# skhu101/SHERF

Hardware: NVIDIA B200
Metric: ray_samples_per_sec (higher is better)
Workload: dtype bf16x3 (bf16 hi/lo split products on tcgen05 kind::f16, 16 significand bits per operand, fp32 accumulate) in every linear layer

## Files before the change

### include/sherf_b200.h

```cpp
#ifndef SHERF_B200_H
#define SHERF_B200_H

#include <stddef.h>
#include <stdint.h>

#ifdef __cplusplus
extern "C" {
#endif

#define SHERF_ABI_VERSION 5
#if defined(__GNUC__)
#define SHERF_API __attribute__((visibility("default")))
#else
#define SHERF_API
#endif
#define SHERF_NUM_JOINTS 24
#define SHERF_NUM_LEVELS 3

enum {
  SHERF_OK = 0,
  SHERF_E_INVALID = -1,
  SHERF_E_SCRATCH = -2,
  SHERF_E_CUDA = -3,
  SHERF_E_UNSUPPORTED = -4
// ... 168 lines not shown
                                                  const SherfInputGrads* grad_inputs, void* scratch, size_t scratch_bytes, void* stream,
                                                  int64_t n_points);

SHERF_API int sherf_depth_range(const SherfRays* rays, float* min_out , float* max_out ,
                      void* scratch, size_t scratch_bytes, void* stream);

SHERF_API int sherf_generate_rays(const double* K, const double* R, const double* T, int32_t H, int32_t W, const double* bounds,
                                  float* origins, float* dirs, float* near_out, float* far_out, uint8_t* mask_at_box ,
                                  void* stream);

#define SHERF_SPARSE_CONVS 13
typedef struct SherfSparseConv {
  const float* weight;
  const float *bn_weight, *bn_bias, *bn_mean, *bn_var;
  int32_t c_in, c_out;
  int32_t kind;
  int32_t reserved;
} SherfSparseConv;
typedef struct SherfSparseEncoder { SherfSparseConv conv[SHERF_SPARSE_CONVS]; } SherfSparseEncoder;

SHERF_API size_t sherf_sparse_encoder_scratch_bytes(int32_t n_voxels, const int32_t* out_sh );
SHERF_API int sherf_sparse_encode(const SherfSparseEncoder* enc, const int32_t* coord, const float* feat, int32_t n,
                                  const int32_t* out_sh , float* vol1, float* vol2, float* vol3, void* scratch,
                                  size_t scratch_bytes, void* stream);

typedef struct SherfSparseEncoderGrads {
  float* weight[SHERF_SPARSE_CONVS];
  float* bn_weight[SHERF_SPARSE_CONVS];
  float* bn_bias[SHERF_SPARSE_CONVS];
} SherfSparseEncoderGrads;
SHERF_API size_t sherf_sparse_encoder_train_scratch_bytes(int32_t n_voxels, const int32_t* out_sh );
SHERF_API int sherf_sparse_encode_train(const SherfSparseEncoder* enc, const int32_t* coord, const float* feat, int32_t n,
                                        const int32_t* out_sh , float* vol1, float* vol2, float* vol3, float* batch_stats,
                                        int32_t* row_counts, int32_t use_running_stats, void* scratch, size_t scratch_bytes, void* stream);
SHERF_API int sherf_sparse_encode_backward(const SherfSparseEncoder* enc, const int32_t* coord, int32_t n, const int32_t* out_sh ,
                                           const float* g_vol1, const float* g_vol2, const float* g_vol3, const SherfSparseEncoderGrads* grads,
                                           float* g_feat, int32_t use_running_stats , void* scratch, size_t scratch_bytes,
                                           void* stream);

typedef struct SherfObservation {
  SherfPose obs;
  SherfPose canonical;
  const float* obs_vertices;
  const float* t_vertices;
  const float* obs_K;
  const float* obs_R;
  const float* obs_T;
  const int32_t* faces;
  const int32_t* last_face;
  int32_t n_faces;
  int32_t reserved;
  const float* obs_img;
  int32_t img_h, img_w;
  const float* obs_feat;
  int32_t feat_ch, feat_h, feat_w;
  int32_t reserved2;
  const float *proj_w, *proj_b;
} SherfObservation;

SHERF_API size_t sherf_observation_scratch_bytes(int32_t n_verts);
SHERF_API int sherf_prepare_observation(const SherfSmplModel* smpl, const SherfObservation* obs, float* vert_feat, int32_t* coord,
                                        uint8_t* vertex_mask, float* bounds, int32_t* out_sh_host, float* canonical_out, void* scratch,
                                        size_t scratch_bytes, void* stream);

SHERF_API int sherf_prepare_observation_backward(const SherfSmplModel* smpl, const SherfObservation* obs, const float* g_vert_feat,
                                                 float* g_proj_w, float* g_proj_b, float* g_obs_feat, void* scratch, size_t scratch_bytes,
                                                 void* stream);

SHERF_API int sherf_debug_sample_importance(const SherfRays* rays, const float* weights, const float* u, float* t_fine_out,
                                            int32_t* bins_out , void* stream);

SHERF_API int sherf_debug_linear(int precision, const float* A, int lda, const float* W, const float* bias, float* Y, int ldy,
                                 int M, int N, int K, int act, void* scratch, size_t scratch_bytes, void* stream);

SHERF_API void sherf_debug_set_trace(long long* device_buf);

SHERF_API const char* sherf_last_error(void);
SHERF_API int sherf_abi_version(void);
SHERF_API int64_t sherf_last_launch_count(void);
SHERF_API int64_t sherf_last_importance_point_count(void);
SHERF_API void sherf_set_profiling(int enabled);
SHERF_API float sherf_last_stage_ms(int stage);
SHERF_API float sherf_last_host_us(int part);

#ifdef __cplusplus
}
#endif
#endif
```

### sherf_b200/_lib.py

```python
from __future__ import annotations

import ctypes as C
import os

from . import build as _build

c_float_p = C.c_void_p
c_int_p = C.c_void_p

MLP_FP32, MLP_TF32, MLP_TF32X3, MLP_BF16X3 = 0, 1, 2, 3
ABI_VERSION = 5


class SherfSmplModel(C.Structure):
    _fields_ = [('v_template', c_float_p), ('shapedirs', c_float_p), ('posedirs', c_float_p), ('j_regressor', c_float_p),
                ('weights', c_float_p), ('parents', C.c_int32 * 24), ('n_verts', C.c_int32)]


class SherfPose(C.Structure):
    _fields_ = [('poses', c_float_p), ('shapes', c_float_p), ('R', c_float_p), ('Th', c_float_p)]


class SherfFrame(C.Structure):
    _fields_ = [('target', SherfPose), ('canonical', SherfPose), ('obs', SherfPose), ('vertices', c_float_p),
                ('t_vertices', c_float_p), ('t_world_bounds', c_float_p), ('obs_K', c_float_p), ('obs_R', c_float_p),
                ('obs_T', c_float_p), ('sp_bounds', c_float_p), ('out_sh', C.c_int32 * 3)]


class SherfScene(C.Structure):
    _fields_ = [('planes', c_float_p), ('plane_ch', C.c_int32), ('plane_h', C.c_int32), ('plane_w', C.c_int32),
                ('obs_img', c_float_p), ('img_h', C.c_int32), ('img_w', C.c_int32),
                ('obs_feat', c_float_p), ('feat_ch', C.c_int32), ('feat_h', C.c_int32), ('feat_w', C.c_int32),
                ('vol', c_float_p * 3), ('vol_ch', C.c_int32 * 3), ('vol_dim', (C.c_int32 * 3) * 3)]


class SherfWeights(C.Structure):
    _fields_ = [('proj_w', c_float_p), ('proj_b', c_float_p), ('reproj_w', c_float_p), ('reproj_b', c_float_p),
                ('ln1_w', c_float_p), ('ln1_b', c_float_p), ('qkv_w', c_float_p), ('attn_out_w', c_float_p),
                ('attn_out_b', c_float_p), ('ln2_w', c_float_p), ('ln2_b', c_float_p), ('ff1_w', c_float_p),
                ('ff1_b', c_float_p), ('ff2_w', c_float_p), ('ff2_b', c_float_p), ('pts_w', c_float_p * 8),
                ('pts_b', c_float_p * 8), ('alpha_w', c_float_p), ('alpha_b', c_float_p), ('feature_w', c_float_p),
                ('feature_b', c_float_p), ('views_w', c_float_p), ('views_b', c_float_p), ('rgb_w', c_float_p),
                ('rgb_b', c_float_p)]


class SherfWeightGrads(C.Structure):
    _fields_ = list(SherfWeights._fields_)


class SherfOutGrads(C.Structure):
    _fields_ = [('rgb', c_float_p), ('depth', c_float_p), ('acc', c_float_p)]


class SherfInputGrads(C.Structure):
    _fields_ = [('planes', c_float_p), ('obs_feat', c_float_p), ('vol', c_float_p * 3)]


class SherfRays(C.Structure):
    _fields_ = [('origins', c_float_p), ('dirs', c_float_p), ('near_', c_float_p), ('far_', c_float_p),
                ('n_rays', C.c_int32), ('n_samples', C.c_int32), ('n_importance', C.c_int32), ('reserved', C.c_int32)]


class SherfOptions(C.Structure):
    _fields_ = [('white_back', C.c_int32), ('mlp_precision', C.c_int32), ('depth_clamp_min', C.c_float),
                ('depth_clamp_max', C.c_float), ('use_external_clamp', C.c_int32), ('density_noise', c_float_p),
                ('importance_u', c_float_p), ('density_noise_importance', c_float_p), ('weights_version', C.c_uint64), ('scene_version', C.c_uint64)]


class SherfOut(C.Structure):
    _fields_ = [('rgb', c_float_p), ('depth', c_float_p), ('acc', c_float_p)]


class SherfDebug(C.Structure):
    _fields_ = [('sample_vid', c_int_p), ('point_sample', c_int_p), ('point_vid3', c_int_p), ('point_can', c_float_p),
                ('point_cdir', c_float_p), ('point_uv', c_float_p), ('point_feat', c_float_p), ('point_tok', c_float_p),
                ('point_sigma', c_float_p), ('point_rgb', c_float_p), ('max_points', C.c_int64), ('max_feat_points', C.c_int64),
                ('coarse_weights', c_float_p), ('fine_depths', c_float_p), ('fine_bins', c_int_p), ('fine_sample_vid', c_int_p),
                ('fine_sigma', c_float_p), ('fine_rgb', c_float_p)]


class SherfSparseConv(C.Structure):
    _fields_ = [('weight', c_float_p), ('bn_weight', c_float_p), ('bn_bias', c_float_p), ('bn_mean', c_float_p), ('bn_var', c_float_p),
                ('c_in', C.c_int32), ('c_out', C.c_int32), ('kind', C.c_int32), ('reserved', C.c_int32)]


class SherfSparseEncoder(C.Structure):
    _fields_ = [('conv', SherfSparseConv * 13)]


class SherfSparseEncoderGrads(C.Structure):
    _fields_ = [('weight', c_float_p * 13), ('bn_weight', c_float_p * 13), ('bn_bias', c_float_p * 13)]


class SherfObservation(C.Structure):
    _fields_ = [('obs', SherfPose), ('canonical', SherfPose), ('obs_vertices', c_float_p), ('t_vertices', c_float_p), ('obs_K', c_float_p),
                ('obs_R', c_float_p), ('obs_T', c_float_p), ('faces', c_int_p), ('last_face', c_int_p), ('n_faces', C.c_int32),
                ('reserved', C.c_int32), ('obs_img', c_float_p), ('img_h', C.c_int32), ('img_w', C.c_int32), ('obs_feat', c_float_p),
                ('feat_ch', C.c_int32), ('feat_h', C.c_int32), ('feat_w', C.c_int32), ('reserved2', C.c_int32), ('proj_w', c_float_p),
                ('proj_b', c_float_p)]


EXPORTS = ['sherf_render_backward_after_forward', 'sherf_sparse_encoder_train_scratch_bytes', 'sherf_sparse_encode_train', 'sherf_sparse_encode_backward', 'sherf_prepare_observation_backward', 'sherf_backward_scratch_bytes', 'sherf_render_backward', 'sherf_smpl_vertices', 'sherf_count_survivors', 'sherf_observation_scratch_bytes', 'sherf_prepare_observation', 'sherf_debug_set_trace', 'sherf_sparse_encoder_scratch_bytes', 'sherf_sparse_encode', 'sherf_generate_rays', 'sherf_debug_sample_importance', 'sherf_debug_linear', 'sherf_scratch_bytes', 'sherf_render_forward', 'sherf_lbs_transforms', 'sherf_depth_range', 'sherf_last_error',
           'sherf_abi_version', 'sherf_last_launch_count', 'sherf_last_importance_point_count', 'sherf_set_profiling', 'sherf_last_stage_ms', 'sherf_last_host_us']

_lib = None


def lib_path() -> str:
    return _build.LIB_PATH


def load():
    global _lib
    if _lib is not None:
        return _lib
    path = lib_path()
    if not os.path.exists(path):
        raise RuntimeError(f'{path} not found: build it with `python -m sherf_b200.build` (or __graft_entry__.build()); '
                           'sherf_b200 has no CPU or PyTorch fallback')
    lib = C.CDLL(path)
    lib.sherf_scratch_bytes.restype = C.c_size_t
    lib.sherf_scratch_bytes.argtypes = [C.POINTER(SherfScene), C.c_int32, C.c_int32, C.c_int32, C.c_int32]
    lib.sherf_render_forward.restype = C.c_int
    lib.sherf_render_forward.argtypes = [C.POINTER(SherfSmplModel), C.POINTER(SherfFrame), C.POINTER(SherfScene),
                                         C.POINTER(SherfWeights), C.POINTER(SherfRays), C.POINTER(SherfOptions),
                                         C.POINTER(SherfOut), C.POINTER(SherfDebug), C.c_void_p, C.c_size_t, C.c_void_p,
                                         C.POINTER(C.c_int64)]
    lib.sherf_backward_scratch_bytes.restype = C.c_size_t
    lib.sherf_backward_scratch_bytes.argtypes = [C.POINTER(SherfScene), C.c_int32, C.c_int32, C.c_int32]
    lib.sherf_render_backward.restype = C.c_int
    lib.sherf_render_backward.argtypes = [C.POINTER(SherfSmplModel), C.POINTER(SherfFrame), C.POINTER(SherfScene),
                                          C.POINTER(SherfWeights), C.POINTER(SherfRays), C.POINTER(SherfOptions),
                                          C.POINTER(SherfOutGrads), C.POINTER(SherfWeightGrads), C.POINTER(SherfInputGrads),
                                          C.c_void_p, C.c_size_t, C.c_void_p, C.POINTER(C.c_int64)]
    lib.sherf_render_backward_after_forward.restype = C.c_int
    lib.sherf_render_backward_after_forward.argtypes = lib.sherf_render_backward.argtypes[:-1] + [C.c_int64]
    lib.sherf_count_survivors.restype = C.c_int
    lib.sherf_count_survivors.argtypes = [C.POINTER(SherfSmplModel), C.POINTER(SherfFrame), C.POINTER(SherfScene), C.POINTER(SherfRays),
                                          C.POINTER(SherfOptions), C.c_void_p, C.c_size_t, C.c_void_p, C.POINTER(C.c_int64)]
    lib.sherf_smpl_vertices.restype = C.c_int
    lib.sherf_smpl_vertices.argtypes = [C.POINTER(SherfSmplModel), C.POINTER(SherfPose), C.c_void_p, C.c_void_p, C.c_void_p, C.c_size_t, C.c_void_p]
    lib.sherf_lbs_transforms.restype = C.c_int
    lib.sherf_lbs_transforms.argtypes = [C.POINTER(SherfSmplModel), C.POINTER(SherfPose), C.c_void_p, C.c_void_p, C.c_size_t,
                                         C.c_void_p]
    lib.sherf_depth_range.restype = C.c_int
    lib.sherf_depth_range.argtypes = [C.POINTER(SherfRays), C.POINTER(C.c_float), C.POINTER(C.c_float), C.c_void_p, C.c_size_t,
                                      C.c_void_p]
    lib.sherf_debug_linear.restype = C.c_int
    lib.sherf_debug_linear.argtypes = [C.c_int, C.c_void_p, C.c_int, C.c_void_p, C.c_void_p, C.c_void_p, C.c_int, C.c_int, C.c_int, C.c_int,
                                       C.c_int, C.c_void_p, C.c_size_t, C.c_void_p]
    lib.sherf_debug_sample_importance.restype = C.c_int
    lib.sherf_debug_sample_importance.argtypes = [C.POINTER(SherfRays), C.c_void_p, C.c_void_p, C.c_void_p, C.c_void_p, C.c_void_p]
    lib.sherf_generate_rays.restype = C.c_int
    lib.sherf_generate_rays.argtypes = [C.POINTER(C.c_double), C.POINTER(C.c_double), C.POINTER(C.c_double), C.c_int32, C.c_int32,
                                        C.POINTER(C.c_double), C.c_void_p, C.c_void_p, C.c_void_p, C.c_void_p, C.c_void_p, C.c_void_p]
    lib.sherf_sparse_encoder_scratch_bytes.restype = C.c_size_t
    lib.sherf_sparse_encoder_scratch_bytes.argtypes = [C.c_int32, C.POINTER(C.c_int32)]
    lib.sherf_sparse_encode.restype = C.c_int
    lib.sherf_sparse_encode.argtypes = [C.POINTER(SherfSparseEncoder), C.c_void_p, C.c_void_p, C.c_int32, C.POINTER(C.c_int32), C.c_void_p, C.c_void_p,
                                        C.c_void_p, C.c_void_p, C.c_size_t, C.c_void_p]
    lib.sherf_sparse_encoder_train_scratch_bytes.restype = C.c_size_t
    lib.sherf_sparse_encoder_train_scratch_bytes.argtypes = [C.c_int32, C.POINTER(C.c_int32)]
    lib.sherf_sparse_encode_train.restype = C.c_int
    lib.sherf_sparse_encode_train.argtypes = [C.POINTER(SherfSparseEncoder), C.c_void_p, C.c_void_p, C.c_int32, C.POINTER(C.c_int32), C.c_void_p,
                                              C.c_void_p, C.c_void_p, C.c_void_p, C.c_void_p, C.c_int32, C.c_void_p, C.c_size_t, C.c_void_p]
    lib.sherf_sparse_encode_backward.restype = C.c_int
    lib.sherf_sparse_encode_backward.argtypes = [C.POINTER(SherfSparseEncoder), C.c_void_p, C.c_int32, C.POINTER(C.c_int32), C.c_void_p, C.c_void_p,
                                                 C.c_void_p, C.POINTER(SherfSparseEncoderGrads), C.c_void_p, C.c_int32, C.c_void_p, C.c_size_t, C.c_void_p]
    lib.sherf_prepare_observation_backward.restype = C.c_int
    lib.sherf_prepare_observation_backward.argtypes = [C.POINTER(SherfSmplModel), C.POINTER(SherfObservation), C.c_void_p, C.c_void_p, C.c_void_p,
                                                       C.c_void_p, C.c_void_p, C.c_size_t, C.c_void_p]
    lib.sherf_observation_scratch_bytes.restype = C.c_size_t
    lib.sherf_observation_scratch_bytes.argtypes = [C.c_int32]
    lib.sherf_prepare_observation.restype = C.c_int
    lib.sherf_prepare_observation.argtypes = [C.POINTER(SherfSmplModel), C.POINTER(SherfObservation), C.c_void_p, C.c_void_p, C.c_void_p,
                                              C.c_void_p, C.POINTER(C.c_int32), C.c_void_p, C.c_void_p, C.c_size_t, C.c_void_p]
    lib.sherf_debug_set_trace.argtypes = [C.c_void_p]
    lib.sherf_last_error.restype = C.c_char_p
    lib.sherf_abi_version.restype = C.c_int
    lib.sherf_last_launch_count.restype = C.c_int64
    lib.sherf_last_importance_point_count.restype = C.c_int64
    lib.sherf_set_profiling.argtypes = [C.c_int]
    lib.sherf_last_stage_ms.restype = C.c_float
    lib.sherf_last_stage_ms.argtypes = [C.c_int]
    lib.sherf_last_host_us.restype = C.c_float
    lib.sherf_last_host_us.argtypes = [C.c_int]
    if lib.sherf_abi_version() != ABI_VERSION:
        raise RuntimeError('libsherf_b200.so ABI version mismatch')
    _lib = lib
    return lib


def check(rc: int):
    if rc != 0:
        raise RuntimeError(f'sherf_b200 error {rc}: {load().sherf_last_error().decode()}')
```

### sherf_b200/csrc/api.cu

```cuda
#include "common.cuh"
#include "stages.cuh"
#include <cstdarg>
#include <cstdio>
#include <cstring>
#include <cstdlib>
#include <vector>
#include <chrono>

namespace sherf {

thread_local LaunchCounter g_launches;
thread_local bool g_pack_plan_only = false;
static thread_local char g_err[512] = "";
static thread_local int64_t g_last_launches = 0;
static thread_local int64_t g_last_fine_points = 0;
static thread_local int g_profiling = 0;
static thread_local float g_stage_ms[8] = {0, 0, 0, 0, 0, 0, 0, 0};
static thread_local float g_host_us[4] = {0, 0, 0, 0};
static inline double now_us() { return std::chrono::duration<double, std::micro>(std::chrono::steady_clock::now().time_since_epoch()).count(); }

void set_error(const char* fmt, ...) {
  va_list ap;
  va_start(ap, fmt);
  vsnprintf(g_err, sizeof(g_err), fmt, ap);
  va_end(ap);
}

constexpr int kMaxCell = 1 << 18;
static size_t chunk_cap_limit() {
  static size_t cap = 0;
  if (!cap) {
    const char* e = getenv("SHERF_CHUNK_CAP");
    const long v = e ? atol(e) : 0;
    cap = v >= 128 ? (size_t)(v / 128 * 128) : (size_t)(1 << 19);
  }
  return cap;
}

struct Arena {
  char* base; size_t size; size_t off; bool dry;
  template <typename T> T* take(size_t n) {
    off = (off + 255) & ~(size_t)255;
    T* p = dry ? nullptr : reinterpret_cast<T*>(base + off);
    off += n * sizeof(T);
    return p;
  }
};

struct Layout {
  FrameTables ft;
  float* planes_cl; float* feat_cl; float* vol_cl[3];
  int* sample_vid; int* ray_count; int* block_sums; int* ray_start; int64_t* total;
  int* point_sample; int* point_vid;
  float* sigma; float* rgb;
  float* fine_depths; int* sample_vid_f; int* ray_count_f; int* ray_start_f; int64_t* total_f; int* point_sample_f; int* point_vid_f;
  float* sigma_f; float* rgb_f;
  float* packed_w;
  float* canon_w;
  unsigned char* fused_blob; float* fused_bias; float* xf_blob; float* ff_blob;
  unsigned char* pp_blob; float* pp_bias; unsigned char* pp_xv;
  unsigned char* xb_blob; unsigned char* fr_blob;
  float* chunk;
  float* gather2;
  float* lbs_joints; float* lbs_pf;
};

static int chunk_cap(int N, int S, int SF) {
  const size_t NS = (size_t)N * (S > SF ? S : SF);
  return (int)((NS < chunk_cap_limit()) ? ((NS + 127) / 128 * 128) : chunk_cap_limit());
}

static size_t carve(Arena& a, const SherfScene& sc, int N, int S, int SF, int V, Layout& L) {
  const size_t NS = (size_t)N * S, NF = (size_t)N * SF;
  FrameTables& ft = L.ft;
  ft.fc = a.take<FrameConst>(1);
  ft.A = a.take<float>(3 * kJoints * 16);
  ft.joints = a.take<float>(3 * kJoints * 3);
  ft.posefeat = a.take<float>(3 * kPoseFeat);
  ft.poff = a.take<float>((size_t)3 * V * 3);
  ft.soff = a.take<float>((size_t)2 * V * 3);
  ft.verts_smpl = a.take<float>((size_t)V * 3);
  ft.T1 = a.take<VertexWarp>(V);
  ft.T3 = a.take<VertexWarp>(V);
  ft.g1_cell_start = a.take<int>(kMaxCell + 1);
  ft.g3_cell_start = a.take<int>(kMaxCell + 1);
  ft.g_cursor = a.take<int>((size_t)2 * kMaxCell);
  ft.g_block_sums = a.take<int>((size_t)2 * (kMaxCell / 1024 + 2));
  ft.g_total = a.take<int64_t>(2);
  ft.g1_verts = a.take<float4>(V);
  ft.g3_verts = a.take<float4>(V);
  ft.g1_occ = a.take<unsigned char>(kMaxCell);
  ft.maxcell = kMaxCell;
  L.lbs_joints = a.take<float>(kJoints * 3);
  L.lbs_pf = a.take<float>(kPoseFeat);
  L.planes_cl = a.take<float>((size_t)3 * sc.plane_ch * sc.plane_h * sc.plane_w);
  L.feat_cl = a.take<float>((size_t)sc.feat_ch * sc.feat_h * sc.feat_w);
  for (int l = 0; l < 3; ++l)
    L.vol_cl[l] = a.take<float>((size_t)sc.vol_ch[l] * sc.vol_dim[l][0] * sc.vol_dim[l][1] * sc.vol_dim[l][2]);
  L.sample_vid = a.take<int>(NS);
  L.ray_count = a.take<int>(N);
  L.block_sums = a.take<int>((size_t)N / 1024 + 2);
  L.ray_start = a.take<int>((size_t)N + 1);
  L.total = a.take<int64_t>(1);
  L.point_sample = a.take<int>(NS);
  L.point_vid = a.take<int>(NS);
  L.sigma = a.take<float>(NS);
  L.rgb = a.take<float>(NS * 3);
  L.fine_depths = nullptr; L.sample_vid_f = nullptr; L.ray_count_f = nullptr; L.ray_start_f = nullptr; L.total_f = nullptr;
  L.point_sample_f = nullptr; L.point_vid_f = nullptr; L.sigma_f = nullptr; L.rgb_f = nullptr;
  if (SF > 0) {
    L.fine_depths = a.take<float>(NF);
    L.sample_vid_f = a.take<int>(NF);
    L.ray_count_f = a.take<int>(N);
    L.ray_start_f = a.take<int>((size_t)N + 1);
    L.total_f = a.take<int64_t>(1);
    L.point_sample_f = a.take<int>(NF);
    L.point_vid_f = a.take<int>(NF);
    L.sigma_f = a.take<float>(NF);
    L.rgb_f = a.take<float>(NF * 3);
  }
  L.packed_w = a.take<float>(packed_weight_floats());
  L.canon_w = a.take<float>(canonical_weight_floats());
  L.fused_blob = a.take<unsigned char>(fused_blob_bytes());
  L.fused_bias = a.take<float>(10 * 144);
  L.xf_blob = a.take<float>(xformer_blob_floats());
  L.ff_blob = a.take<float>(fusion_blob_floats());
  const int cap = chunk_cap(N, S, SF);
  L.chunk = a.take<float>(chunk_buffer_floats(cap));
  L.pp_blob = a.take<unsigned char>(pp_blob_bytes());
  L.pp_bias = a.take<float>(10 * 128);
  L.pp_xv = a.take<unsigned char>(pp_xv_bytes(cap));
  L.gather2 = a.take<float>((size_t)cap * (288 + 192 + 8));
  L.xb_blob = a.take<unsigned char>(xformer_bf16_blob_bytes());
  L.fr_blob = a.take<unsigned char>(front_blob_bytes());
  return a.off;
}

struct StageTimer {
  struct Span { int stage; cudaEvent_t a, b; cudaStream_t s; };
  std::vector<Span> spans; bool on = false; cudaStream_t st = nullptr;
  std::vector<int> open_stack;
  static std::vector<cudaEvent_t>& pool() { static thread_local std::vector<cudaEvent_t> p; return p; }
  size_t used = 0;
  cudaEvent_t get_event() {
    auto& p = pool();
    if (used == p.size()) { cudaEvent_t e; cudaEventCreate(&e); p.push_back(e); }
    return p[used++];
  }
  void init(bool enable, cudaStream_t s) { on = enable; st = s; used = 0; }
  void begin(int stage, cudaStream_t on_stream = nullptr) {
    if (!on) return;
    Span sp; sp.stage = stage; sp.s = on_stream ? on_stream : st;
    sp.a = get_event(); sp.b = get_event();
    cudaEventRecord(sp.a, sp.s);
    spans.push_back(sp);
    open_stack.push_back((int)spans.size() - 1);
  }
  void end() {
    if (!on || open_stack.empty()) return;
    cudaEventRecord(spans[open_stack.back()].b, spans[open_stack.back()].s);
    open_stack.pop_back();
  }
  void finish() {
    if (!on) return;
    for (int i = 0; i < 8; ++i) g_stage_ms[i] = 0.f;
    cudaStreamSynchronize(st);
    for (auto& sp : spans) {
      float ms = 0.f;
      cudaEventElapsedTime(&ms, sp.a, sp.b);
      g_stage_ms[sp.stage] += ms;
    }
    spans.clear();
  }
};

static thread_local StageTimer* g_tm = nullptr;

struct PackTag { const void* base = nullptr; size_t need = 0; uint64_t version = 0; int precision = -1; int dev = -1; uint64_t scene = 0; };
static thread_local PackTag g_pack_tag;

static int64_t* pinned_counts() {
  static thread_local int64_t* p = nullptr;
  if (!p && cudaHostAlloc((void**)&p, 4 * sizeof(int64_t), cudaHostAllocDefault) != cudaSuccess) p = nullptr;
  return p;
}

static cudaEvent_t count_event(int which) {
  static thread_local cudaEvent_t ev[2] = {nullptr, nullptr};
  static thread_local int dev = -1;
  int d = 0;
  if (cudaGetDevice(&d) != cudaSuccess) return nullptr;
  if (d != dev) { ev[0] = ev[1] = nullptr; dev = d; }
  if (!ev[which] && cudaEventCreateWithFlags(&ev[which], cudaEventDisableTiming) != cudaSuccess) ev[which] = nullptr;
  return ev[which];
}

struct SideStream {
  cudaStream_t s = nullptr; cudaEvent_t fork = nullptr, ldone = nullptr, gdone[2] = {nullptr, nullptr}, mdone[2] = {nullptr, nullptr}; int dev = -1;
  int ensure() {
    int d = 0;
    if (cudaGetDevice(&d) != cudaSuccess) return -1;
    if (s && d == dev) return 0;
    dev = d;
    int lo = 0, hi = 0;
    cudaDeviceGetStreamPriorityRange(&lo, &hi);
    if (cudaStreamCreateWithPriority(&s, cudaStreamNonBlocking, hi) != cudaSuccess) return -1;
    cudaEventCreateWithFlags(&fork, cudaEventDisableTiming);
    cudaEventCreateWithFlags(&ldone, cudaEventDisableTiming);
    for (int i = 0; i < 2; ++i) { cudaEventCreateWithFlags(&gdone[i], cudaEventDisableTiming); cudaEventCreateWithFlags(&mdone[i], cudaEventDisableTiming); }
    return 0;
  }
};
static thread_local SideStream g_side;
static void fill_gather_params(GatherParams& G, const SherfRays& rays, const SherfFrame& frame, const SherfScene& scene, const Layout& L) {
  G.origins = rays.origins; G.dirs = rays.dirs; G.nearv = rays.near_; G.farv = rays.far_; G.S = rays.n_samples; G.depths = nullptr;
  G.point_sample = L.point_sample; G.point_vid = L.point_vid; G.p0 = 0; G.np = 0; G.dc = DevCount{nullptr, 0, 0};
  G.fc = L.ft.fc; G.T1 = L.ft.T1; G.T3 = L.ft.T3; G.g3_start = L.ft.g3_cell_start; G.g3_verts = L.ft.g3_verts;
  G.t_vertices = getenv("SHERF_KNN3_UNSEEDED") ? nullptr : frame.t_vertices;
  G.planes_cl = L.planes_cl; G.plane_h = scene.plane_h; G.plane_w = scene.plane_w;
  G.feat_cl = L.feat_cl; G.feat_h = scene.feat_h; G.feat_w = scene.feat_w; G.feat_ch = scene.feat_ch;
  G.img = scene.obs_img; G.img_h = scene.img_h; G.img_w = scene.img_w;
  for (int l = 0; l < 3; ++l) {
    G.vol_cl[l] = L.vol_cl[l]; G.vol_ch[l] = scene.vol_ch[l];
    G.vol_d[l] = scene.vol_dim[l][0]; G.vol_h[l] = scene.vol_dim[l][1]; G.vol_w[l] = scene.vol_dim[l][2];
  }
  G.comb = nullptr; G.f3raw = nullptr; G.geo = nullptr;
  G.g_planes_cl = nullptr; G.g_feat_cl = nullptr; G.g_vol_cl[0] = G.g_vol_cl[1] = G.g_vol_cl[2] = nullptr;
  G.dbg_vid3 = nullptr; G.dbg_can = nullptr; G.dbg_cdir = nullptr; G.dbg_uv = nullptr; G.dbg_feat = nullptr; G.dbg_max = 0; G.dbg_feat_max = 0;
}

struct BwdLayout {
  float* out;
  float* dsig; float* drgb;
  float* g_planes_cl; float* g_feat_cl; float* g_vol_cl[3];
  float* canon_w; float* canon_bwd;
  float* chunk; int bcap;
};
static int bwd_chunk_cap(int N, int S) {
  const char* e = getenv("SHERF_BWD_CHUNK_CAP");
  const long v = e ? atol(e) : 0;
  const int cap = v >= 128 ? (int)(v / 128 * 128) : (1 << 20);
  const size_t NS = (size_t)N * S;
  return (int)(NS < (size_t)cap ? (NS + 127) / 128 * 128 : (size_t)cap);
}
static size_t carve_backward(Arena& a, const SherfScene& sc, int N, int S, int V, Layout& L, BwdLayout& B, size_t* fwd_need) {
  const size_t f = carve(a, sc, N, S, 0, V, L);
  if (fwd_need) *fwd_need = f;
  const size_t NS = (size_t)N * S;
  B.out = a.take<float>((size_t)5 * N);
  B.dsig = a.take<float>(NS);
  B.drgb = a.take<float>(NS * 3);
  B.g_planes_cl = a.take<float>((size_t)3 * sc.plane_ch * sc.plane_h * sc.plane_w);
  B.g_feat_cl = a.take<float>((size_t)sc.feat_ch * sc.feat_h * sc.feat_w);
  for (int l = 0; l < 3; ++l) B.g_vol_cl[l] = a.take<float>((size_t)sc.vol_ch[l] * sc.vol_dim[l][0] * sc.vol_dim[l][1] * sc.vol_dim[l][2]);
  B.canon_w = a.take<float>(canonical_weight_floats());
  B.canon_bwd = a.take<float>(canonical_bwd_weight_floats());
  B.bcap = bwd_chunk_cap(N, S);
  B.chunk = a.take<float>(bwd_chunk_floats(B.bcap));
  return a.off;
}

static void nested_begin(int stage) { if (g_tm) g_tm->begin(stage); }
static void nested_end() { if (g_tm) g_tm->end(); }

}

using namespace sherf;

extern "C" {

int sherf_abi_version(void) { return SHERF_ABI_VERSION; }
const char* sherf_last_error(void) { return g_err; }
int64_t sherf_last_launch_count(void) { return g_last_launches; }
int64_t sherf_last_importance_point_count(void) { return g_last_fine_points; }
void sherf_set_profiling(int enabled) { g_profiling = enabled; }
float sherf_last_stage_ms(int stage) { return (stage >= 0 && stage < 8) ? g_stage_ms[stage] : 0.f; }
float sherf_last_host_us(int part) { return (part >= 0 && part < 4) ? g_host_us[part] : 0.f; }

size_t sherf_scratch_bytes(const SherfScene* scene, int32_t n_rays, int32_t n_samples, int32_t n_importance, int32_t n_verts) {
  if (!scene || n_rays <= 0 || n_samples < 2 || n_importance < 0 || n_verts <= 0) return 0;
  Arena a{nullptr, 0, 0, true};
  Layout L;
  return carve(a, *scene, n_rays, n_samples, n_importance, n_verts, L) + 512;
}

static int validate(const SherfSmplModel* smpl, const SherfFrame* fr, const SherfScene* sc, const SherfWeights* w,
                    const SherfRays* rays, const SherfOptions* opts, const SherfOut* out) {
  if (!smpl || !fr || !sc || !w || !rays || !opts || !out) { set_error("null argument struct"); return SHERF_E_INVALID; }
  if (rays->n_rays <= 0 || rays->n_samples < 2 || rays->n_samples > 256) {
    set_error("n_rays must be > 0 and 2 <= n_samples <= 256 (got %d, %d)", rays->n_rays, rays->n_samples);
    return SHERF_E_INVALID;
  }
  if ((int64_t)rays->n_rays * rays->n_samples >= (1LL << 31)) { set_error("n_rays * n_samples must be < 2^31"); return SHERF_E_INVALID; }
  if (rays->n_importance < 0 || rays->n_importance > 256) { set_error("n_importance must be in 0..256 (got %d)", rays->n_importance); return SHERF_E_INVALID; }
  if (rays->n_importance > 0) {
    if (rays->n_samples < 3) { set_error("the importance pass needs n_samples >= 3 (sample_pdf bins, renderer.py:498-499)"); return SHERF_E_INVALID; }
    if (!opts->importance_u) { set_error("n_importance > 0 needs SherfOptions.importance_u (the torch.rand draws of renderer.py:526)"); return SHERF_E_INVALID; }
    const int64_t smax = rays->n_samples > rays->n_importance ? rays->n_samples : rays->n_importance;
    if ((int64_t)rays->n_rays * smax >= (1LL << 30)) { set_error("n_rays * max(n_samples, n_importance) must be < 2^30 with the importance pass"); return SHERF_E_INVALID; }
  }
  if (sc->plane_ch != 32 || sc->feat_ch != 64 || sc->vol_ch[0] != 32 || sc->vol_ch[1] != 64 || sc->vol_ch[2] != 96) {
    set_error("unsupported channel counts (planes %d, feat %d, volumes %d/%d/%d; expected 32, 64, 32/64/96)", sc->plane_ch,
              sc->feat_ch, sc->vol_ch[0], sc->vol_ch[1], sc->vol_ch[2]);
    return SHERF_E_UNSUPPORTED;
  }
  if (opts->mlp_precision < SHERF_MLP_FP32 || opts->mlp_precision > SHERF_MLP_BF16X3) { set_error("unknown mlp_precision %d", opts->mlp_precision); return SHERF_E_UNSUPPORTED; }
  if (!rays->origins || !rays->dirs || !rays->near_ || !rays->far_ || !out->rgb || !out->depth || !out->acc || !sc->planes ||
      !sc->obs_img || !sc->obs_feat || !sc->vol[0] || !sc->vol[1] || !sc->vol[2] || !smpl->weights || !smpl->posedirs) {
    set_error("null device pointer in arguments");
    return SHERF_E_INVALID;
  }
  {
    const SherfPose* poses[3] = {&fr->target, &fr->canonical, &fr->obs};
    bool ok = fr->vertices && fr->t_vertices && fr->t_world_bounds && fr->obs_K && fr->obs_R && fr->obs_T && fr->sp_bounds && smpl->v_template &&
              smpl->shapedirs && smpl->j_regressor;
    for (int i = 0; i < 3; ++i) ok = ok && poses[i]->poses && poses[i]->shapes;
    ok = ok && fr->target.R && fr->target.Th && fr->obs.R && fr->obs.Th;
    const float* const* wp = reinterpret_cast<const float* const*>(w);
    for (size_t i = 0; i < sizeof(SherfWeights) / sizeof(const float*); ++i) ok = ok && wp[i] != nullptr;
    if (!ok) { set_error("null device pointer in SherfFrame / SherfSmplModel / SherfWeights"); return SHERF_E_INVALID; }
  }
  return SHERF_OK;
}

#define RC(x) do { int _rc = (x); if (_rc) return _rc; } while (0)

int sherf_render_forward(const SherfSmplModel* smpl, const SherfFrame* frame, const SherfScene* scene,
                         const SherfWeights* weights, const SherfRays* rays, const SherfOptions* opts, const SherfOut* out,
                         const SherfDebug* dbg, void* scratch, size_t scratch_bytes, void* stream, int64_t* n_points_out) {
  g_err[0] = 0;
  const double t_enter = now_us();
  RC(validate(smpl, frame, scene, weights, rays, opts, out));
  const int N = rays->n_rays, S = rays->n_samples, SF = rays->n_importance, V = smpl->n_verts;
  cudaStream_t st = (cudaStream_t)stream;
  Arena a{(char*)scratch, scratch_bytes, 0, false};
  const size_t mis = ((size_t)a.base) & 255;
  if (mis) { a.base += 256 - mis; a.size -= 256 - mis; }
  Layout L;
  const size_t need = carve(a, *scene, N, S, SF, V, L);
  if (!scratch || need > a.size) { set_error("scratch arena too small: need %zu bytes, have %zu", need, scratch_bytes); return SHERF_E_SCRATCH; }
  g_launches.n = 0;
  g_last_fine_points = 0;
  StageTimer tm;
  tm.init(g_profiling != 0, st);
  g_tm = &tm;
  struct Guard {
    cudaStream_t st; bool forked = false, joined = false;
    ~Guard() {
      g_tm = nullptr;
      if (forked && !joined && g_side.s) { cudaEventRecord(g_side.ldone, g_side.s); cudaStreamWaitEvent(st, g_side.ldone, 0); }
    }
  } guard;
  guard.st = st;

  const bool side = !getenv("SHERF_NO_PROLOGUE_OVERLAP") && g_side.ensure() == 0;
  cudaStream_t ls = side ? g_side.s : st;
  tm.begin(0);
  RC(run_prologue_frame(*frame, L.ft, st));
  if (side) { SHERF_CUDA_OK(cudaEventRecord(g_side.fork, st)); SHERF_CUDA_OK(cudaStreamWaitEvent(ls, g_side.fork, 0)); guard.forked = true; }
  RC(run_prologue_cull(*smpl, *frame, *rays, *opts, L.ft, st));
// ... 82 lines not shown
    G.S = Sn; G.depths = depths; G.point_sample = point_sample; G.point_vid = point_vid; G.p0 = p0; G.np = np; G.dc = dc;
    G.comb = cbi.comb; G.f3raw = cbi.f3raw; G.geo = cbi.geo;
    G.dbg_vid3 = d ? d->point_vid3 : nullptr; G.dbg_can = d ? d->point_can : nullptr;
    G.dbg_cdir = d ? d->point_cdir : nullptr; G.dbg_uv = d ? d->point_uv : nullptr;
    G.dbg_feat = d ? d->point_feat : nullptr; G.dbg_max = d ? d->max_points : 0;
    G.dbg_feat_max = d ? d->max_feat_points : 0;
    if (overlap && ci >= 2) SHERF_CUDA_OK(cudaStreamWaitEvent(gs, g_side.mdone[bsel], 0));
    tm.begin(2, gs);
    if (fplan.fr_blob) RC(run_front_fused(G, *weights, fplan.fr_blob, cbi.tok, gs));
    else RC(run_point_gather(G, gs));
    tm.end();
    if (overlap) { SHERF_CUDA_OK(cudaEventRecord(g_side.gdone[bsel], gs)); SHERF_CUDA_OK(cudaStreamWaitEvent(st, g_side.gdone[bsel], 0)); }
    tm.begin(3);
    RC(run_mlp(opts->mlp_precision, *weights, pw, cw, use_fused ? &fplan : nullptr, cbi, np, p0, sigma_out, rgb_out, d ? d->point_tok : nullptr,
               d ? d->max_points : 0, st, nested_begin, nested_end, dc));
    tm.end();
    if (overlap) SHERF_CUDA_OK(cudaEventRecord(g_side.mdone[bsel], st));
    return SHERF_OK;
  };
  auto run_points = [&](const int* point_sample, const int* point_vid, int64_t Pn, int64_t first_p0, int Sn, const float* depths, float* sigma_out,
                        float* rgb_out, const SherfDebug* d) -> int {
    const bool overlap = first_p0 == 0 && Pn > cb.cap && getenv("SHERF_OVERLAP") && g_side.ensure() == 0;
    cudaStream_t gs = overlap ? g_side.s : st;
    if (overlap) { SHERF_CUDA_OK(cudaEventRecord(g_side.fork, st)); SHERF_CUDA_OK(cudaStreamWaitEvent(gs, g_side.fork, 0)); }
    int ci = (int)(first_p0 / cb.cap);
    for (int64_t p0 = first_p0; p0 < Pn; p0 += cb.cap, ++ci) {
      const int np = (int)((Pn - p0 < cb.cap) ? (Pn - p0) : cb.cap);
      RC(issue_chunk(point_sample, point_vid, p0, np, Sn, depths, sigma_out, rgb_out, d, DevCount{nullptr, 0, 0}, ci, overlap, gs));
    }
    return SHERF_OK;
  };
  const bool async_first = fplan.fr_blob && fplan.xb_blob && use_pp && !dbg && !getenv("SHERF_SYNC_FIRST_CHUNK");
  if (side) { SHERF_CUDA_OK(cudaStreamWaitEvent(st, g_side.ldone, 0)); guard.joined = true; }
  if (async_first)
    RC(issue_chunk(L.point_sample, L.point_vid, 0, cb.cap, S, nullptr, L.sigma, L.rgb, nullptr, DevCount{L.total, 0, cb.cap}, 0, false, st));
  const double t_sync0 = now_us();
  SHERF_CUDA_OK(cudaEventSynchronize(ev_cnt0));
  const int64_t P = hcount[0];
  const double t_sync1 = now_us();
  if (n_points_out) *n_points_out = P;
  if (dbg && dbg->point_sample && P > 0)
    SHERF_CUDA_OK(cudaMemcpyAsync(dbg->point_sample, L.point_sample, sizeof(int) * (size_t)(P < dbg->max_points ? P : dbg->max_points),
                                  cudaMemcpyDeviceToDevice, st));
  RC(run_points(L.point_sample, L.point_vid, P, async_first ? cb.cap : 0, S, nullptr, L.sigma, L.rgb, dbg));
  if (dbg && P > 0) {
    const size_t cnt = (size_t)(P < dbg->max_points ? P : dbg->max_points);
    if (dbg->point_sigma) SHERF_CUDA_OK(cudaMemcpyAsync(dbg->point_sigma, L.sigma, sizeof(float) * cnt, cudaMemcpyDeviceToDevice, st));
    if (dbg->point_rgb) SHERF_CUDA_OK(cudaMemcpyAsync(dbg->point_rgb, L.rgb, sizeof(float) * 3 * cnt, cudaMemcpyDeviceToDevice, st));
  }

  if (SF == 0) {
    tm.begin(4);
    RC(run_composite(*rays, L.ft.fc, L.ray_start, L.point_sample, L.sigma, L.rgb, opts->density_noise, opts->white_back, *out, st));
    tm.end();
  } else {
    tm.begin(4);
    RC(run_importance_sample(*rays, L.ray_start, L.point_sample, L.sigma, opts->density_noise, nullptr, opts->importance_u, L.fine_depths,
                             dbg ? dbg->fine_bins : nullptr, dbg ? dbg->coarse_weights : nullptr, st));
    tm.end();
    tm.begin(1);
    int* vid_f = (dbg && dbg->fine_sample_vid) ? dbg->fine_sample_vid : L.sample_vid_f;
    RC(run_cull(*rays, SF, L.fine_depths, L.ft, vid_f, L.ray_count_f, L.block_sums, L.ray_start_f, L.total_f, L.point_sample_f, L.point_vid_f, st));
    tm.end();
    SHERF_CUDA_OK(cudaMemcpyAsync(&hcount[1], L.total_f, sizeof(int64_t), cudaMemcpyDeviceToHost, st));
    SHERF_CUDA_OK(cudaEventRecord(ev_cnt1, st));
    if (async_first)
      RC(issue_chunk(L.point_sample_f, L.point_vid_f, 0, cb.cap, SF, L.fine_depths, L.sigma_f, L.rgb_f, nullptr, DevCount{L.total_f, 0, cb.cap}, 0, false, st));
    SHERF_CUDA_OK(cudaEventSynchronize(ev_cnt1));
    const int64_t PF = hcount[1];
    if (n_points_out) *n_points_out = P + PF;
    g_last_fine_points = PF;
    RC(run_points(L.point_sample_f, L.point_vid_f, PF, async_first ? cb.cap : 0, SF, L.fine_depths, L.sigma_f, L.rgb_f, nullptr));
    if (dbg) {
      if (dbg->fine_depths) SHERF_CUDA_OK(cudaMemcpyAsync(dbg->fine_depths, L.fine_depths, sizeof(float) * (size_t)N * SF, cudaMemcpyDeviceToDevice, st));
      RC(run_dense_taps(L.point_sample_f, L.sigma_f, L.rgb_f, PF, (int64_t)N * SF, dbg->fine_sigma, dbg->fine_rgb, st));
    }
    tm.begin(4);
    RC(run_composite_merged(*rays, L.ft.fc, sample_vid, L.ray_start, L.sigma, L.rgb, opts->density_noise, L.fine_depths, vid_f, L.ray_start_f,
                            L.sigma_f, L.rgb_f, opts->density_noise_importance, opts->white_back, *out, st));
    tm.end();
  }
  tm.finish();
  g_last_launches = g_launches.n;
  { const double t_exit = now_us(); g_host_us[0] = (float)(t_sync0 - t_enter); g_host_us[1] = (float)(t_sync1 - t_sync0); g_host_us[2] = (float)(t_exit - t_sync1); g_host_us[3] = (float)(t_exit - t_enter); }
  return SHERF_OK;
}

size_t sherf_backward_scratch_bytes(const SherfScene* scene, int32_t n_rays, int32_t n_samples, int32_t n_verts) {
  if (!scene || n_rays <= 0 || n_samples < 2 || n_verts <= 0) return 0;
  Arena a{nullptr, 0, 0, true};
  Layout L;
  BwdLayout B;
  return carve_backward(a, *scene, n_rays, n_samples, n_verts, L, B, nullptr) + 512;
}

static int render_backward_impl(const SherfSmplModel* smpl, const SherfFrame* frame, const SherfScene* scene, const SherfWeights* weights,
                                const SherfRays* rays, const SherfOptions* opts, const SherfOutGrads* grad_out, const SherfWeightGrads* grad_weights,
                                const SherfInputGrads* grad_inputs, void* scratch, size_t scratch_bytes, void* stream, int64_t* n_points_out,
                                int64_t forward_points );

int sherf_render_backward(const SherfSmplModel* smpl, const SherfFrame* frame, const SherfScene* scene, const SherfWeights* weights,
                          const SherfRays* rays, const SherfOptions* opts, const SherfOutGrads* grad_out, const SherfWeightGrads* grad_weights,
                          const SherfInputGrads* grad_inputs, void* scratch, size_t scratch_bytes, void* stream, int64_t* n_points_out) {
  return render_backward_impl(smpl, frame, scene, weights, rays, opts, grad_out, grad_weights, grad_inputs, scratch, scratch_bytes, stream, n_points_out, -1);
}

int sherf_render_backward_after_forward(const SherfSmplModel* smpl, const SherfFrame* frame, const SherfScene* scene, const SherfWeights* weights,
                                        const SherfRays* rays, const SherfOptions* opts, const SherfOutGrads* grad_out,
                                        const SherfWeightGrads* grad_weights, const SherfInputGrads* grad_inputs, void* scratch, size_t scratch_bytes,
                                        void* stream, int64_t n_points) {
  if (n_points < 0) { g_err[0] = 0; set_error("n_points must be the survivor count the forward reported"); return SHERF_E_INVALID; }
  return render_backward_impl(smpl, frame, scene, weights, rays, opts, grad_out, grad_weights, grad_inputs, scratch, scratch_bytes, stream, nullptr, n_points);
}

}

static int render_backward_impl(const SherfSmplModel* smpl, const SherfFrame* frame, const SherfScene* scene, const SherfWeights* weights,
                                const SherfRays* rays, const SherfOptions* opts, const SherfOutGrads* grad_out, const SherfWeightGrads* grad_weights,
                                const SherfInputGrads* grad_inputs, void* scratch, size_t scratch_bytes, void* stream, int64_t* n_points_out,
                                int64_t forward_points) {
  g_err[0] = 0;
  if (!smpl || !frame || !scene || !weights || !rays || !opts || !grad_out || !scratch) { set_error("null argument"); return SHERF_E_INVALID; }
  if (rays->n_importance != 0) {
    set_error("sherf_render_backward covers the coarse pass only (n_importance must be 0; the reference's fine pass cannot execute, SURVEY a13)");
    return SHERF_E_UNSUPPORTED;
  }
  const int N = rays->n_rays, S = rays->n_samples, V = smpl->n_verts;
  if (N <= 0 || S < 2 || V <= 0) { set_error("bad sizes"); return SHERF_E_INVALID; }
  cudaStream_t st = (cudaStream_t)stream;
  Arena a{(char*)scratch, scratch_bytes, 0, false};
  const size_t mis = ((size_t)a.base) & 255;
  if (mis) { a.base += 256 - mis; a.size -= 256 - mis; }
  Layout L;
  BwdLayout B;
  size_t fwd_need = 0;
  const size_t need = carve_backward(a, *scene, N, S, V, L, B, &fwd_need);
  if (need > a.size) { set_error("backward scratch arena too small: need %zu bytes, have %zu", need, scratch_bytes); return SHERF_E_SCRATCH; }

  SherfOut fout; fout.rgb = B.out; fout.depth = B.out + (size_t)3 * N; fout.acc = B.out + (size_t)4 * N;
  int64_t P = forward_points;
  int64_t launches = 0;
  if (forward_points < 0) {
    RC(sherf_render_forward(smpl, frame, scene, weights, rays, opts, &fout, nullptr, a.base, fwd_need + 256, stream, &P));
    launches = g_launches.n;
  } else if (forward_points > (int64_t)N * S) { set_error("n_points exceeds n_rays * n_samples"); return SHERF_E_INVALID; }
  if (n_points_out) *n_points_out = P;
  g_launches.n = 0;

  SherfWeightGrads gw;
  if (grad_weights) gw = *grad_weights; else memset(&gw, 0, sizeof(gw));
  {
    float* const* gp = reinterpret_cast<float* const*>(&gw);
    const int n_out[20] = {96, 32, 32, 144, 32, 32, 32, 32, 128, 128, 128, 128, 128, 128, 128, 128, 1, 128, 64, 3};
    const int n_in[20] = {192, 96, 0, 32, 48, 0, 32, 32, 71, 128, 128, 128, 128, 199, 128, 128, 128, 128, 187, 64};
    size_t sizes[39]; int k = 0;
    auto wb = [&](int layer, bool bias) { sizes[k++] = (size_t)n_out[layer] * (n_in[layer] ? n_in[layer] : 1); if (bias) sizes[k++] = n_out[layer]; };
    wb(0, true); wb(1, true);
    sizes[k++] = 32; sizes[k++] = 32;
    wb(3, false); wb(4, true);
    sizes[k++] = 32; sizes[k++] = 32;
    wb(6, true); wb(7, true);
    for (int i = 0; i < 8; ++i) sizes[k++] = (size_t)128 * n_in[8 + i];
    for (int i = 0; i < 8; ++i) sizes[k++] = 128;
    wb(16, true); wb(17, true); wb(18, true); wb(19, true);
    if (k != 39 || sizeof(SherfWeightGrads) != 39 * sizeof(float*)) { set_error("internal: weight table mismatch"); return SHERF_E_INVALID; }
    for (int i = 0; i < 39; ++i)
      if (gp[i]) SHERF_CUDA_OK(cudaMemsetAsync(gp[i], 0, sizes[i] * sizeof(float), st));
  }
  const bool want_planes = grad_inputs && grad_inputs->planes, want_feat = grad_inputs && grad_inputs->obs_feat;
  bool want_vol[3];
  for (int l = 0; l < 3; ++l) want_vol[l] = grad_inputs && grad_inputs->vol[l];
  const size_t plane = (size_t)scene->plane_ch * scene->plane_h * scene->plane_w;
  if (want_planes) SHERF_CUDA_OK(cudaMemsetAsync(B.g_planes_cl, 0, 3 * plane * sizeof(float), st));
  if (want_feat) SHERF_CUDA_OK(cudaMemsetAsync(B.g_feat_cl, 0, (size_t)scene->feat_ch * scene->feat_h * scene->feat_w * sizeof(float), st));
  size_t vol_n[3];
  for (int l = 0; l < 3; ++l) {
    vol_n[l] = (size_t)scene->vol_ch[l] * scene->vol_dim[l][0] * scene->vol_dim[l][1] * scene->vol_dim[l][2];
    if (want_vol[l]) SHERF_CUDA_OK(cudaMemsetAsync(B.g_vol_cl[l], 0, vol_n[l] * sizeof(float), st));
  }

  if (P > 0) {
    PackedWeights pw;
    g_pack_plan_only = false;
    RC(run_pack_weights(*weights, L.packed_w, pw, st));
    CanonWeights cw;
    CanonBwdWeights cbw;
    RC(run_pack_canonical(*weights, B.canon_w, cw, st));
    RC(run_pack_canonical_bwd(*weights, B.canon_bwd, cbw, st));
    RC(run_composite_backward(*rays, L.ft.fc, L.ray_start, L.point_sample, L.sigma, L.rgb, opts->density_noise, opts->white_back, grad_out->rgb,
                              grad_out->depth, grad_out->acc, B.dsig, B.drgb, st));
    BwdChunk bc;
    carve_bwd_chunk(B.chunk, B.bcap, bc);
    GatherParams G;
    fill_gather_params(G, *rays, *frame, *scene, L);
    for (int64_t p0 = 0; p0 < P; p0 += B.bcap) {
      const int np = (int)((P - p0 < B.bcap) ? (P - p0) : B.bcap);
      RC(run_backward_chunk(*weights, pw, cw, cbw, gw, G, bc, np, p0, L.rgb, B.dsig, B.drgb, st));
      GatherParams Gs = G;
      Gs.g_planes_cl = want_planes ? B.g_planes_cl : nullptr;
      Gs.g_feat_cl = want_feat ? B.g_feat_cl : nullptr;
      for (int l = 0; l < 3; ++l) Gs.g_vol_cl[l] = want_vol[l] ? B.g_vol_cl[l] : nullptr;
      RC(run_backward_chunk_inputs(*weights, cbw, Gs, bc, np, p0, st));
    }
  }
  if (want_planes)
    for (int k = 0; k < 3; ++k)
      RC(run_from_channels_last(B.g_planes_cl + k * plane, grad_inputs->planes + k * plane, scene->plane_ch, (int64_t)scene->plane_h * scene->plane_w, st));
  if (want_feat) RC(run_from_channels_last(B.g_feat_cl, grad_inputs->obs_feat, scene->feat_ch, (int64_t)scene->feat_h * scene->feat_w, st));
  for (int l = 0; l < 3; ++l)
    if (want_vol[l])
      RC(run_from_channels_last(B.g_vol_cl[l], grad_inputs->vol[l], scene->vol_ch[l], (int64_t)(vol_n[l] / scene->vol_ch[l]), st));
  g_last_launches = launches + g_launches.n;
  return SHERF_OK;
}

extern "C" {

int sherf_count_survivors(const SherfSmplModel* smpl, const SherfFrame* frame, const SherfScene* scene, const SherfRays* rays, const SherfOptions* opts,
                          void* scratch, size_t scratch_bytes, void* stream, int64_t* n_points_out) {
  g_err[0] = 0;
  if (!smpl || !frame || !scene || !rays || !opts || !scratch || !n_points_out) { set_error("null argument"); return SHERF_E_INVALID; }
  if (rays->n_rays <= 0 || rays->n_samples < 2 || rays->n_samples > 256 || !rays->origins || !rays->dirs || !rays->near_ || !rays->far_) {
    set_error("bad rays"); return SHERF_E_INVALID;
  }
  const int N = rays->n_rays, S = rays->n_samples, SF = rays->n_importance, V = smpl->n_verts;
  cudaStream_t st = (cudaStream_t)stream;
  Arena a{(char*)scratch, scratch_bytes, 0, false};
  const size_t mis = ((size_t)a.base) & 255;
  if (mis) { a.base += 256 - mis; a.size -= 256 - mis; }
  Layout L;
  const size_t need = carve(a, *scene, N, S, SF, V, L);
  if (need > a.size) { set_error("scratch arena too small: need %zu bytes, have %zu", need, scratch_bytes); return SHERF_E_SCRATCH; }
  g_launches.n = 0;
  RC(run_prologue_frame(*frame, L.ft, st));
  RC(run_prologue_cull(*smpl, *frame, *rays, *opts, L.ft, st));
  RC(run_cull(*rays, S, nullptr, L.ft, L.sample_vid, L.ray_count, L.block_sums, L.ray_start, L.total, L.point_sample, L.point_vid, st));
  int64_t* hcount = pinned_counts();
  if (!hcount) { set_error("cudaHostAlloc failed for the survivor-count words"); return SHERF_E_CUDA; }
  SHERF_CUDA_OK(cudaMemcpyAsync(&hcount[2], L.total, sizeof(int64_t), cudaMemcpyDeviceToHost, st));
  SHERF_CUDA_OK(cudaStreamSynchronize(st));
  *n_points_out = hcount[2];
  g_last_launches = g_launches.n;
  return SHERF_OK;
}

int sherf_debug_sample_importance(const SherfRays* rays, const float* weights, const float* u, float* t_fine_out, int32_t* bins_out,
                                  void* stream) {
  g_err[0] = 0;
  if (!rays || !weights || !u || !t_fine_out || !rays->near_ || !rays->far_) { set_error("null argument"); return SHERF_E_INVALID; }
  if (rays->n_rays <= 0 || rays->n_samples < 3 || rays->n_samples > 256 || rays->n_importance < 1 || rays->n_importance > 256) {
    set_error("need n_rays > 0, 3 <= n_samples <= 256, 1 <= n_importance <= 256");
    return SHERF_E_INVALID;
  }
  g_launches.n = 0;
  RC(run_importance_sample(*rays, nullptr, nullptr, nullptr, nullptr, weights, u, t_fine_out, bins_out, nullptr, (cudaStream_t)stream));
  g_last_launches = g_launches.n;
  return SHERF_OK;
}

int sherf_generate_rays(const double* K, const double* R, const double* T, int32_t H, int32_t W, const double* bounds, float* origins,
                        float* dirs, float* near_out, float* far_out, uint8_t* mask_at_box, void* stream) {
  g_err[0] = 0;
  if (!K || !R || !T || !bounds || !origins || !dirs || !near_out || !far_out) { set_error("null argument"); return SHERF_E_INVALID; }
  if (H <= 0 || W <= 0 || (int64_t)H * W >= (1LL << 31)) { set_error("bad image size %d x %d", H, W); return SHERF_E_INVALID; }
  g_launches.n = 0;
  RC(run_generate_rays(K, R, T, H, W, bounds, origins, dirs, near_out, far_out, mask_at_box, (cudaStream_t)stream));
  g_last_launches = g_launches.n;
  return SHERF_OK;
}

size_t sherf_sparse_encoder_scratch_bytes(int32_t n_voxels, const int32_t* out_sh) {
  if (n_voxels <= 0 || !out_sh || out_sh[0] <= 0 || out_sh[1] <= 0 || out_sh[2] <= 0) return 0;
  return sparse_encoder_scratch_bytes(n_voxels, out_sh);
}

int sherf_sparse_encode(const SherfSparseEncoder* enc, const int32_t* coord, const float* feat, int32_t n, const int32_t* out_sh, float* vol1,
                        float* vol2, float* vol3, void* scratch, size_t scratch_bytes, void* stream) {
// ... 182 lines not shown
```

### sherf_b200/csrc/common.cuh

```cuda
#pragma once
#include <cuda_runtime.h>
#include <stdint.h>
#include <stddef.h>
#include <string.h>
#include "../../include/sherf_b200.h"

namespace sherf {

constexpr int kJoints = 24;
constexpr int kPoseFeat = 207;
constexpr float kPi2 = 1.57079632679489661923f;

struct GridDesc {
  float origin[3];
  float inv_cell;
  float cell;
  int dim[3];
  int ncell;
};

struct __align__(16) VertexWarp {
  float Rinv[9];
  float t[3];
  float off0[3];
  float off1[3];
  float off2[3];
  float Af[12];
  float pad[3];
};
static_assert(sizeof(VertexWarp) == 36 * 4, "VertexWarp must be 144 B");

struct FrameConst {
  float R_tgt[9], Th_tgt[3];
  float Rinv_obs[9], Th_obs[3];
  float camR[9], camT[3], camK[9];
  float twb_min[3], twb_max[3];
  float spb_min[3];
  float out_sh[3];
  GridDesc g1, g3;
  int dmin_bits, dmax_bits;
  float dmin, dmax;
};

__host__ __device__ inline int float_to_ordered(float f) {
#ifdef __CUDA_ARCH__
  int i = __float_as_int(f);
#else
  int i; memcpy(&i, &f, 4);
#endif
  return i >= 0 ? i : i ^ 0x7fffffff;
}
__device__ inline float ordered_to_float(int i) { return __int_as_float(i >= 0 ? i : i ^ 0x7fffffff); }

__device__ __forceinline__ float sample_depth(float nearv, float farv, int i, int S) {
  float step = __fdiv_rn((float)i, (float)(S - 1));
  return __fadd_rn(nearv, __fmul_rn(step, __fsub_rn(farv, nearv)));
}
__device__ __forceinline__ float mul_add_sep(float a, float b, float c) {
  return __fadd_rn(c, __fmul_rn(a, b));
}
__device__ __forceinline__ void rowvec_mat3(const float p[3], const float* __restrict__ M, float out[3]) {
#pragma unroll
  for (int j = 0; j < 3; ++j)
    out[j] = __fmaf_rn(p[2], M[6 + j], __fmaf_rn(p[1], M[3 + j], __fmul_rn(p[0], M[j])));
}
__device__ __forceinline__ float dist2_xyz(float qx, float qy, float qz, float vx, float vy, float vz) {
  float dx = __fsub_rn(qx, vx), dy = __fsub_rn(qy, vy), dz = __fsub_rn(qz, vz);
  return __fadd_rn(__fadd_rn(__fmul_rn(dx, dx), __fmul_rn(dy, dy)), __fmul_rn(dz, dz));
}
__device__ __forceinline__ int grid_coord(float x, float origin, float inv_cell, int dim) {
  int c = (int)floorf((x - origin) * inv_cell);
  return c;
}

__device__ __forceinline__ void mat3_vec(const float* __restrict__ M, const float v[3], float out[3]) {
#pragma unroll
  for (int i = 0; i < 3; ++i) out[i] = M[3 * i] * v[0] + M[3 * i + 1] * v[1] + M[3 * i + 2] * v[2];
}

struct LaunchCounter { int64_t n = 0; };
extern thread_local LaunchCounter g_launches;
void set_error(const char* fmt, ...);
extern thread_local bool g_pack_plan_only;

#define SHERF_CUDA_OK(expr)                                                              \
  do {                                                                                   \
    cudaError_t _e = (expr);                                                             \
    if (_e != cudaSuccess) {                                                             \
      ::sherf::set_error("%s failed: %s (%s:%d)", #expr, cudaGetErrorString(_e), __FILE__, __LINE__); \
      return SHERF_E_CUDA;                                                               \
    }                                                                                    \
  } while (0)

#define SHERF_LAUNCH_CHECK()                                                             \
  do {                                                                                   \
    ::sherf::g_launches.n++;                                                             \
    cudaError_t _e = cudaGetLastError();                                                 \
    if (_e != cudaSuccess) {                                                             \
      ::sherf::set_error("kernel launch failed: %s (%s:%d)", cudaGetErrorString(_e), __FILE__, __LINE__); \
      return SHERF_E_CUDA;                                                               \
    }                                                                                    \
  } while (0)

inline int ceil_div(int64_t a, int64_t b) { return (int)((a + b - 1) / b); }

struct FrameTables {
  FrameConst* fc;
  float* A;
  float* joints;
  float* posefeat;
  float* poff;
  float* soff;
  float* verts_smpl;
  VertexWarp* T1;
  VertexWarp* T3;
  int* g1_cell_start;
  int* g3_cell_start;
  int* g_cursor;
  int* g_block_sums;
  int64_t* g_total;
  float4* g1_verts;
  float4* g3_verts;
  unsigned char* g1_occ;
  int maxcell;
};

int run_prologue_frame(const SherfFrame& frame, const FrameTables& ft, cudaStream_t st);
int run_prologue_cull(const SherfSmplModel& smpl, const SherfFrame& frame, const SherfRays& rays, const SherfOptions& opts,
                      const FrameTables& ft, cudaStream_t st);
int run_prologue_tables(const SherfSmplModel& smpl, const SherfFrame& frame, const FrameTables& ft, cudaStream_t st);
int run_lbs_only(const SherfSmplModel& smpl, const SherfPose& pose, float* A_out, float* joints_tmp, float* pf_tmp, cudaStream_t st);
int run_depth_range(const SherfRays& rays, FrameConst* fc, cudaStream_t st);
int run_exclusive_scan(const int* cnt, int n, int* block_sums, int* start, int64_t* total_dev, cudaStream_t st);

}
```

### sherf_b200/csrc/cull.cu

```cuda
#include "common.cuh"

namespace sherf {

__device__ __forceinline__ void nn_27(const GridDesc& g, const int* __restrict__ cell_start, const float4* __restrict__ gv,
                                      float qx, float qy, float qz, int cx, int cy, int cz, float& best, int& best_id) {
  const int x0 = max(cx - 1, 0), x1 = min(cx + 1, g.dim[0] - 1);
  for (int z = max(cz - 1, 0); z <= min(cz + 1, g.dim[2] - 1); ++z) {
    for (int y = max(cy - 1, 0); y <= min(cy + 1, g.dim[1] - 1); ++y) {
      const int row = (z * g.dim[1] + y) * g.dim[0];
      const int b = cell_start[row + x0], e = cell_start[row + x1 + 1];
      for (int k = b; k < e; ++k) {
        const float4 v = gv[k];
        const float d2 = dist2_xyz(qx, qy, qz, v.x, v.y, v.z);
        const int id = __float_as_int(v.w);
        if (d2 < best || (d2 == best && id < best_id)) { best = d2; best_id = id; }
      }
    }
  }
}

__device__ __forceinline__ void cull_query(const FrameConst& fc, const float* __restrict__ origins, const float* __restrict__ dirs, int n,
                                           float t, float q[3]) {
  float p[3];
  p[0] = __fsub_rn(mul_add_sep(t, dirs[n * 3], origins[n * 3]), fc.Th_tgt[0]);
  p[1] = __fsub_rn(mul_add_sep(t, dirs[n * 3 + 1], origins[n * 3 + 1]), fc.Th_tgt[1]);
  p[2] = __fsub_rn(mul_add_sep(t, dirs[n * 3 + 2], origins[n * 3 + 2]), fc.Th_tgt[2]);
  rowvec_mat3(p, fc.R_tgt, q);
}

__global__ void __launch_bounds__(256) k_cull_candidates(const float* __restrict__ origins, const float* __restrict__ dirs,
                                                         const float* __restrict__ nearv, const float* __restrict__ farv, int N, int S,
                                                         const FrameConst* __restrict__ fcp, const unsigned char* __restrict__ occ,
                                                         const float* __restrict__ depths, int* __restrict__ sample_vid,
                                                         int* __restrict__ ray_count, int* __restrict__ queue, int* __restrict__ queue_count,
                                                         int write_all) {
  __shared__ FrameConst fc;
  for (int i = threadIdx.x; i < (int)(sizeof(FrameConst) / 4); i += blockDim.x) ((int*)&fc)[i] = ((const int*)fcp)[i];
  __syncthreads();
  const int lane = threadIdx.x & 31;
  const int n = blockIdx.x * (blockDim.x >> 5) + (threadIdx.x >> 5);
  if (n >= N) return;
  const float nr = nearv[n], fr = farv[n];
  const GridDesc& g = fc.g1;
  if (lane == 0) ray_count[n] = 0;
  float t0 = -3.0e38f, t1 = 3.0e38f;
  {
    float po[3] = {origins[n * 3] - fc.Th_tgt[0], origins[n * 3 + 1] - fc.Th_tgt[1], origins[n * 3 + 2] - fc.Th_tgt[2]};
    float pd[3] = {dirs[n * 3], dirs[n * 3 + 1], dirs[n * 3 + 2]}, qo[3], qd[3];
    rowvec_mat3(po, fc.R_tgt, qo);
    rowvec_mat3(pd, fc.R_tgt, qd);
    const float tmag = fmaxf(fabsf(nr), fabsf(fr));
#pragma unroll
    for (int k = 0; k < 3; ++k) {
      const float margin = 1.0e-3f + 1.0e-5f * (fabsf(qo[k]) + tmag * fabsf(qd[k]));
      const float lo = g.origin[k] - margin, hi = g.origin[k] + (float)g.dim[k] * g.cell + margin;
      if (fabsf(qd[k]) < 1.0e-12f) {
        if (qo[k] < lo || qo[k] > hi) { t0 = 1.f; t1 = 0.f; }
      } else {
        const float a = (lo - qo[k]) / qd[k], b = (hi - qo[k]) / qd[k];
        t0 = fmaxf(t0, fminf(a, b));
        t1 = fminf(t1, fmaxf(a, b));
      }
    }
    const float slack = 1.0e-5f * (fabsf(t0) + fabsf(t1)) + 1.0e-6f;
    t0 -= slack; t1 += slack;
  }
  const bool ray_misses = !(t0 <= t1) || t1 < fminf(nr, fr) || t0 > fmaxf(nr, fr);
  if (ray_misses && !write_all && !depths) return;
  for (int i0 = 0; i0 < S; i0 += 32) {
    const int i = i0 + lane;
    bool cand = false;
    if (i < S) {
      const float t = depths ? depths[(size_t)n * S + i] : sample_depth(nr, fr, i, S);
      float q[3];
      if (t < t0 || t > t1) { sample_vid[(size_t)n * S + i] = -1; }
      else {
      cull_query(fc, origins, dirs, n, t, q);
      const int cx = grid_coord(q[0], g.origin[0], g.inv_cell, g.dim[0]);
      const int cy = grid_coord(q[1], g.origin[1], g.inv_cell, g.dim[1]);
      const int cz = grid_coord(q[2], g.origin[2], g.inv_cell, g.dim[2]);
      cand = cx >= 0 && cx < g.dim[0] && cy >= 0 && cy < g.dim[1] && cz >= 0 && cz < g.dim[2] && occ[(cz * g.dim[1] + cy) * g.dim[0] + cx];
      if (!cand) sample_vid[(size_t)n * S + i] = -1;
      }
    }
    const unsigned m = __ballot_sync(0xffffffffu, cand);
    if (m) {
      int base = 0;
      if (lane == 0) base = atomicAdd(queue_count, __popc(m));
      base = __shfl_sync(0xffffffffu, base, 0);
      if (cand) queue[base + __popc(m & ((1u << lane) - 1u))] = n * S + i;
    }
  }
}

__global__ void __launch_bounds__(256) k_cull_search(const float* __restrict__ origins, const float* __restrict__ dirs,
                                                     const float* __restrict__ nearv, const float* __restrict__ farv, int S,
                                                     const FrameConst* __restrict__ fcp, const int* __restrict__ cell_start,
                                                     const float4* __restrict__ gv, float thr, const float* __restrict__ depths,
                                                     const int* __restrict__ queue, const int* __restrict__ queue_count,
                                                     int* __restrict__ sample_vid, int* __restrict__ ray_count) {
  __shared__ FrameConst fc;
  for (int i = threadIdx.x; i < (int)(sizeof(FrameConst) / 4); i += blockDim.x) ((int*)&fc)[i] = ((const int*)fcp)[i];
  __syncthreads();
  const GridDesc& g = fc.g1;
  const int count = *queue_count;
  for (int j = blockIdx.x * blockDim.x + threadIdx.x; j < count; j += gridDim.x * blockDim.x) {
    const int s = queue[j];
    const int n = s / S, i = s - n * S;
    const float t = depths ? depths[s] : sample_depth(nearv[n], farv[n], i, S);
    float q[3];
    cull_query(fc, origins, dirs, n, t, q);
    const int cx = grid_coord(q[0], g.origin[0], g.inv_cell, g.dim[0]);
    const int cy = grid_coord(q[1], g.origin[1], g.inv_cell, g.dim[1]);
    const int cz = grid_coord(q[2], g.origin[2], g.inv_cell, g.dim[2]);
    float best = 3.0e38f;
    int bid = 0x7fffffff;
    nn_27(g, cell_start, gv, q[0], q[1], q[2], cx, cy, cz, best, bid);
    const int vid = best < thr ? bid : -1;
    sample_vid[s] = vid;
    if (vid >= 0) atomicAdd(&ray_count[n], 1);
  }
}

__global__ void __launch_bounds__(1024) k_ray_block_sums(const int* __restrict__ cnt, int N, int* __restrict__ bsum) {
  __shared__ int red[32];
  const int i = blockIdx.x * 1024 + threadIdx.x;
  int v = i < N ? cnt[i] : 0;
  for (int o = 16; o > 0; o >>= 1) v += __shfl_xor_sync(0xffffffffu, v, o);
  if ((threadIdx.x & 31) == 0) red[threadIdx.x >> 5] = v;
  __syncthreads();
  if (threadIdx.x < 32) {
    int x = red[threadIdx.x];
    for (int o = 16; o > 0; o >>= 1) x += __shfl_xor_sync(0xffffffffu, x, o);
    if (threadIdx.x == 0) bsum[blockIdx.x] = x;
  }
}

__global__ void __launch_bounds__(1024) k_scan_rays(const int* __restrict__ cnt, const int* __restrict__ bsum, int nblocks, int N,
                                                    int* __restrict__ start, int64_t* total_out) {
  __shared__ int red[32];
  __shared__ int warp_off[32];
  __shared__ int block_off;
  const int tid = threadIdx.x, lane = tid & 31, w = tid >> 5;
  int pre = 0;
  for (int b = tid; b < (int)blockIdx.x; b += 1024) pre += bsum[b];
  for (int o = 16; o > 0; o >>= 1) pre += __shfl_xor_sync(0xffffffffu, pre, o);
  if (lane == 0) red[w] = pre;
  __syncthreads();
  if (tid < 32) {
    int x = red[tid];
    for (int o = 16; o > 0; o >>= 1) x += __shfl_xor_sync(0xffffffffu, x, o);
    if (tid == 0) block_off = x;
  }
  __syncthreads();
  const int i = blockIdx.x * 1024 + tid;
  const int v = i < N ? cnt[i] : 0;
  int incl = v;
  for (int o = 1; o < 32; o <<= 1) { const int t = __shfl_up_sync(0xffffffffu, incl, o); if (lane >= o) incl += t; }
  __syncthreads();
  if (lane == 31) red[w] = incl;
  __syncthreads();
  if (tid < 32) {
    const int x = red[tid];
    int y = x;
    for (int o = 1; o < 32; o <<= 1) { const int t = __shfl_up_sync(0xffffffffu, y, o); if (tid >= o) y += t; }
    warp_off[tid] = y - x;
  }
  __syncthreads();
  const int excl = block_off + warp_off[w] + incl - v;
  if (i < N) start[i] = excl;
  if (i == N - 1) { start[N] = excl + v; *total_out = excl + v; }
}

__global__ void __launch_bounds__(256) k_compact(const int* __restrict__ sample_vid, const int* __restrict__ ray_start, int N, int S,
                                                 int* __restrict__ point_sample, int* __restrict__ point_vid) {
  const int lane = threadIdx.x & 31;
  const int n = blockIdx.x * (blockDim.x >> 5) + (threadIdx.x >> 5);
  if (n >= N) return;
  int pos = ray_start[n];
  if (ray_start[n + 1] == pos) return;
  for (int i0 = 0; i0 < S; i0 += 32) {
    const int i = i0 + lane;
    const int vid = (i < S) ? sample_vid[(size_t)n * S + i] : -1;
    const unsigned m = __ballot_sync(0xffffffffu, vid >= 0);
    if (vid >= 0) {
      const int p = pos + __popc(m & ((1u << lane) - 1u));
      point_sample[p] = n * S + i;
      point_vid[p] = vid;
    }
    pos += __popc(m);
  }
}

int run_exclusive_scan(const int* cnt, int n, int* block_sums, int* start, int64_t* total_dev, cudaStream_t st) {
  const int nb = ceil_div(n, 1024);
  k_ray_block_sums<<<nb, 1024, 0, st>>>(cnt, n, block_sums);
  SHERF_LAUNCH_CHECK();
  k_scan_rays<<<nb, 1024, 0, st>>>(cnt, block_sums, nb, n, start, total_dev);
  SHERF_LAUNCH_CHECK();
  return SHERF_OK;
}

#define RC_SCAN(x) do { int _rc = (x); if (_rc) return _rc; } while (0)

int run_cull(const SherfRays& rays, int S, const float* depths, const FrameTables& ft, int* sample_vid, int* ray_count, int* block_sums,
             int* ray_start, int64_t* total_dev, int* point_sample, int* point_vid, cudaStream_t st, int write_all) {
  const int N = rays.n_rays;
  const float thr = (float)(0.05 * 0.05);
  int* queue = point_sample;
  int* queue_count = reinterpret_cast<int*>(total_dev);
  SHERF_CUDA_OK(cudaMemsetAsync(queue_count, 0, sizeof(int), st));
  k_cull_candidates<<<ceil_div(N, 8), 256, 0, st>>>(rays.origins, rays.dirs, rays.near_, rays.far_, N, S, ft.fc, ft.g1_occ, depths,
                                                    sample_vid, ray_count, queue, queue_count, write_all);
  SHERF_LAUNCH_CHECK();
  k_cull_search<<<148 * 8, 256, 0, st>>>(rays.origins, rays.dirs, rays.near_, rays.far_, S, ft.fc, ft.g1_cell_start, ft.g1_verts, thr, depths,
                                         queue, queue_count, sample_vid, ray_count);
  SHERF_LAUNCH_CHECK();
  RC_SCAN(run_exclusive_scan(ray_count, N, block_sums, ray_start, total_dev, st));
  k_compact<<<ceil_div(N, 8), 256, 0, st>>>(sample_vid, ray_start, N, S, point_sample, point_vid);
  SHERF_LAUNCH_CHECK();
  return SHERF_OK;
}

}
```

### sherf_b200/csrc/front_fused.cu

```cuda
#include "common.cuh"
#include "stages.cuh"
#include "umma.cuh"
#include <cuda_bf16.h>
#include <cstdlib>

namespace sherf {

namespace fr {
constexpr uint32_t kLboA = 2080;
constexpr uint32_t kChunkHalf = 4 * kLboA;
constexpr uint32_t kChunk = 2 * kChunkHalf;
constexpr int kSlots = 3;
constexpr uint32_t kLboF = 2048;
constexpr uint32_t kF3d = kSlots * kChunk;
constexpr uint32_t kWr = kF3d + 12 * kLboF;
constexpr uint32_t kWrBlock = 4096;
constexpr uint32_t kWp = kWr + 3 * kWrBlock;
constexpr uint32_t kWpStage = 12288;
constexpr uint32_t kSmemBytes = kWp + 2 * kWpStage;
constexpr uint32_t kD1 = 0, kD2 = 96, kF3dLo = 192;
constexpr int kThreads = 512;
}

struct FrontArgs {
  GatherParams G;
  const unsigned char* wblob;
  const float *bp, *br;
  float* tok;
  int knock;
};

__device__ __forceinline__ void fr_arrive(uint64_t* bar) {
  asm volatile("mbarrier.arrive.shared::cta.b64 _, [%0];" ::"r"(umma::smem_u32(bar)) : "memory");
}

__device__ __forceinline__ void fr_apply_warp(const VertexWarp* __restrict__ Tp, float p[3], float d[3], bool with_dir) {
  const float4* r4 = reinterpret_cast<const float4*>(Tp);
  float w[36];
#pragma unroll
  for (int i = 0; i < 9; ++i) { float4 v = r4[i]; w[4 * i] = v.x; w[4 * i + 1] = v.y; w[4 * i + 2] = v.z; w[4 * i + 3] = v.w; }
  float a[3] = {p[0] - w[9], p[1] - w[10], p[2] - w[11]};
  float c[3];
  mat3_vec(w, a, c);
#pragma unroll
  for (int k = 0; k < 3; ++k) { c[k] = c[k] + w[12 + k]; c[k] = c[k] + w[15 + k]; c[k] = c[k] + w[18 + k]; }
  const float* Af = w + 21;
#pragma unroll
  for (int k = 0; k < 3; ++k) p[k] = (Af[4 * k] * c[0] + Af[4 * k + 1] * c[1] + Af[4 * k + 2] * c[2]) + Af[4 * k + 3];
  if (with_dir) {
    float e[3];
    mat3_vec(w, d, e);
#pragma unroll
    for (int k = 0; k < 3; ++k) d[k] = Af[4 * k] * e[0] + Af[4 * k + 1] * e[1] + Af[4 * k + 2] * e[2];
  }
}

__device__ __forceinline__ void fr_grp_lexmin(float& d, int& id) {
#pragma unroll
  for (int o = 2; o > 0; o >>= 1) {
    const float od = __shfl_xor_sync(0xffffffffu, d, o);
    const int oi = __shfl_xor_sync(0xffffffffu, id, o);
    if (od < d || (od == d && oi < id)) { d = od; id = oi; }
  }
}

__device__ __forceinline__ int fr_nn_seeded4(const GridDesc& g, const int* __restrict__ cell_start, const float4* __restrict__ gv,
                                             const float* __restrict__ t_vertices, float qx, float qy, float qz, int l4, int seed) {
  float best = dist2_xyz(qx, qy, qz, t_vertices[seed * 3], t_vertices[seed * 3 + 1], t_vertices[seed * 3 + 2]);
  int bid = seed;
  const float rb = sqrtf(best) * 1.0001f + 1.0e-4f * g.cell;
  const int x0 = min(max(grid_coord(qx - rb, g.origin[0], g.inv_cell, g.dim[0]), 0), g.dim[0] - 1);
  const int x1 = min(max(grid_coord(qx + rb, g.origin[0], g.inv_cell, g.dim[0]), 0), g.dim[0] - 1);
  const int y0 = min(max(grid_coord(qy - rb, g.origin[1], g.inv_cell, g.dim[1]), 0), g.dim[1] - 1);
  const int y1 = min(max(grid_coord(qy + rb, g.origin[1], g.inv_cell, g.dim[1]), 0), g.dim[1] - 1);
  const int z0 = min(max(grid_coord(qz - rb, g.origin[2], g.inv_cell, g.dim[2]), 0), g.dim[2] - 1);
  const int z1 = min(max(grid_coord(qz + rb, g.origin[2], g.inv_cell, g.dim[2]), 0), g.dim[2] - 1);
  const int nx = x1 - x0 + 1, ny = y1 - y0 + 1, ncells = nx * ny * (z1 - z0 + 1);
  for (int cc = l4; cc < ncells; cc += 4) {
    const int xx = x0 + cc % nx, t = cc / nx;
    const int cell = ((z0 + t / ny) * g.dim[1] + (y0 + t % ny)) * g.dim[0] + xx;
    const int b = cell_start[cell], e = cell_start[cell + 1];
    for (int k = b; k < e; ++k) {
      const float4 v = gv[k];
      const float d2 = dist2_xyz(qx, qy, qz, v.x, v.y, v.z);
      const int id = __float_as_int(v.w);
      if (d2 < best || (d2 == best && id < bid)) { best = d2; bid = id; }
    }
  }
  fr_grp_lexmin(best, bid);
  return bid;
}

template <bool DBG>
__global__ void __launch_bounds__(fr::kThreads, 2) k_front_fused(const FrontArgs a) {
  extern __shared__ __align__(128) unsigned char smem[];
  __shared__ FrameConst fc;
  __shared__ __align__(8) uint64_t a_full[fr::kSlots], a_free[fr::kSlots], w_full[2], w_free[2], acc1, acc2, f3d_ready;
  __shared__ uint32_t tmem_base_s;
  __shared__ float s_bp[96], s_br[32];
  __shared__ float s_pt[128][6];
  const GatherParams& P = a.G;
  const int tid = threadIdx.x, warp = tid >> 5, lane = tid & 31, l4 = lane & 3, gbase = lane & 28;
  const int c8 = 8 * l4;

  for (int i = tid; i < (int)(sizeof(FrameConst) / 4); i += blockDim.x) ((int*)&fc)[i] = ((const int*)P.fc)[i];
  if (tid == 0) {
    for (int b = 0; b < fr::kSlots; ++b) { umma::mbar_init(&a_full[b], fr::kThreads); umma::mbar_init(&a_free[b], 1); }
    for (int b = 0; b < 2; ++b) { umma::mbar_init(&w_full[b], 1); umma::mbar_init(&w_free[b], 1); }
    umma::mbar_init(&acc1, 1); umma::mbar_init(&acc2, 1); umma::mbar_init(&f3d_ready, fr::kThreads);
    umma::fence_mbar_init();
  }
  if (warp == 0) umma::tmem_alloc(&tmem_base_s, 256);
  for (int i = tid; i < (int)(3 * fr::kWrBlock / 16); i += blockDim.x)
    reinterpret_cast<uint4*>(smem + fr::kWr)[i] = __ldg(reinterpret_cast<const uint4*>(a.wblob + 6 * fr::kWpStage) + i);
  if (tid < 96) s_bp[tid] = a.bp[tid];
  if (tid < 32) s_br[tid] = a.br[tid];
  umma::fence_proxy_async_smem();
  umma::tc_fence_before_sync();
  __syncthreads();
  umma::tc_fence_after_sync();
  const uint32_t tmem_base = tmem_base_s;
  const uint32_t sbase = umma::smem_u32(smem);
  const int np = resolve_np(P.np, P.dc);
  const int ntiles = (np + 127) / 128;
  const uint32_t el = umma::elect_one();
  const int gi = warp * 8 + (lane >> 2);
  const int erow = 32 * (warp & 3) + lane, ecg = warp >> 2;
  const uint32_t etb = tmem_base + ((uint32_t)(32 * (warp & 3)) << 16);

  if (warp == 0 && lane == 0 && (int)blockIdx.x < ntiles) {
    for (int s = 0; s < 2; ++s) {
      umma::mbar_arrive_expect_tx(&w_full[s], fr::kWpStage);
      umma::bulk_g2s(smem + fr::kWp + s * fr::kWpStage, a.wblob + (size_t)s * fr::kWpStage, fr::kWpStage, &w_full[s]);
    }
  }

  auto gemm32 = [&](uint32_t a_hi_addr, uint32_t a_lbo, bool lo_in_tmem, uint32_t a_lo, uint32_t w_hi_addr, uint32_t w_lo_addr, int N, uint32_t dcol,
                    uint32_t acc0) {
    const uint32_t idesc = umma::make_idesc_bf16(128, N);
    const uint32_t w_lbo = (uint32_t)N * 16u;
    const uint64_t ah0 = umma::make_smem_desc(a_hi_addr, a_lbo, 128u);
    const uint64_t al0 = umma::make_smem_desc(a_lo, a_lbo, 128u);
    const uint64_t wh0 = umma::make_smem_desc(w_hi_addr, w_lbo, 128u);
    const uint64_t wl0 = umma::make_smem_desc(w_lo_addr, w_lbo, 128u);
    const uint64_t da = (uint64_t)((2u * a_lbo) >> 4), dw = (uint64_t)((2u * w_lbo) >> 4);
#pragma unroll
    for (int st = 0; st < 2; ++st) {
      const uint32_t acc = st == 0 ? acc0 : 1u;
      if (lo_in_tmem) umma::mma_bf16_ts_e(tmem_base + dcol, tmem_base + a_lo + (uint32_t)st * 8u, wh0 + (uint64_t)st * dw, idesc, acc, el);
      else umma::mma_bf16_ss_e(tmem_base + dcol, al0 + (uint64_t)st * da, wh0 + (uint64_t)st * dw, idesc, acc, el);
      umma::mma_bf16_ss_e(tmem_base + dcol, ah0 + (uint64_t)st * da, wl0 + (uint64_t)st * dw, idesc, 1u, el);
      umma::mma_bf16_ss_e(tmem_base + dcol, ah0 + (uint64_t)st * da, wh0 + (uint64_t)st * dw, idesc, 1u, el);
    }
  };

  uint32_t ti = 0;
  for (int tile = blockIdx.x; tile < ntiles; tile += gridDim.x, ++ti) {
    const bool has_next = tile + (int)gridDim.x < ntiles;
    bool act;
    int64_t gpt;
    float pu, pv;
    {
      const int lp_raw = tile * 128 + gi;
      act = lp_raw < np;
      const int lp = act ? lp_raw : np - 1;
      const int64_t gp = P.p0 + lp;
      gpt = gp;
      const int s = P.point_sample[gp];
      const int n = s / P.S, i = s - n * P.S;
      const float t = P.depths ? P.depths[s] : sample_depth(P.nearv[n], P.farv[n], i, P.S);
      float dray[3] = {P.dirs[n * 3], P.dirs[n * 3 + 1], P.dirs[n * 3 + 2]};
      float pw[3], q[3], vd[3];
#pragma unroll
      for (int k = 0; k < 3; ++k) pw[k] = __fsub_rn(mul_add_sep(t, dray[k], P.origins[n * 3 + k]), fc.Th_tgt[k]);
      rowvec_mat3(pw, fc.R_tgt, q);
      rowvec_mat3(dray, fc.R_tgt, vd);
      float cn[3] = {q[0], q[1], q[2]}, cdir[3] = {vd[0], vd[1], vd[2]};
      const int vid1 = P.point_vid[gp];
      if (!(a.knock & 8)) fr_apply_warp(P.T1 + vid1, cn, cdir, true);
      const int vid3 = (a.knock & 1) ? vid1 : fr_nn_seeded4(fc.g3, P.g3_start, P.g3_verts, P.t_vertices, cn[0], cn[1], cn[2], l4, vid1);
      float ps[3] = {cn[0], cn[1], cn[2]}, dummy[3] = {0.f, 0.f, 0.f};
      fr_apply_warp(P.T3 + vid3, ps, dummy, false);
      float world[3], cam[3], pix[3];
#pragma unroll
      for (int k = 0; k < 3; ++k) world[k] = (ps[0] * fc.Rinv_obs[k] + ps[1] * fc.Rinv_obs[3 + k] + ps[2] * fc.Rinv_obs[6 + k]) + fc.Th_obs[k];
      mat3_vec(fc.camR, world, cam);
#pragma unroll
      for (int k = 0; k < 3; ++k) cam[k] += fc.camT[k];
      mat3_vec(fc.camK, cam, pix);
      const float zz = pix[2] + 1e-5f;
      const float u = pix[0] / zz, v = pix[1] / zz;
      {
        const int k3 = l4 < 3 ? l4 : 0;
        const float ck = k3 == 0 ? cn[0] : (k3 == 1 ? cn[1] : cn[2]);
        const float gnv = ((ck - fc.spb_min[k3]) / 0.005f) / fc.out_sh[2 - k3] * 2.f - 1.f;
        const float cnv = 2.f * (ck - fc.twb_min[k3]) / (fc.twb_max[k3] - fc.twb_min[k3]) - 1.f;
        if (l4 < 3) { s_pt[gi][l4] = gnv; s_pt[gi][3 + l4] = cnv; }
        pu = u; pv = v;
      }
      if (act) {
        if (l4 < 3) {
          P.geo[(size_t)lp * 8 + l4] = l4 == 0 ? cn[0] : (l4 == 1 ? cn[1] : cn[2]);
          P.geo[(size_t)lp * 8 + 3 + l4] = l4 == 0 ? cdir[0] : (l4 == 1 ? cdir[1] : cdir[2]);
        } else {
          P.geo[(size_t)lp * 8 + 6] = 0.f;
          P.geo[(size_t)lp * 8 + 7] = 0.f;
        }
        if (DBG && l4 == 0 && gp < P.dbg_max) {
          if (P.dbg_vid3) P.dbg_vid3[gp] = vid3;
          if (P.dbg_can) { P.dbg_can[gp * 3] = cn[0]; P.dbg_can[gp * 3 + 1] = cn[1]; P.dbg_can[gp * 3 + 2] = cn[2]; }
          if (P.dbg_cdir) { P.dbg_cdir[gp * 3] = cdir[0]; P.dbg_cdir[gp * 3 + 1] = cdir[1]; P.dbg_cdir[gp * 3 + 2] = cdir[2]; }
          if (P.dbg_uv) { P.dbg_uv[gp * 2] = u; P.dbg_uv[gp * 2 + 1] = v; }
        }
      }
    }
    __syncwarp();

    int offT[2] = {-1, -1}, offI = -1;
    float wT[2] = {0.f, 0.f}, wI = 0.f;
    const float* pt = s_pt[gi];
#pragma unroll 1
    for (int c = 0; c < 12; ++c) {
      if (c == 0 || c == 1 || c == 3) {
        const int l = c == 0 ? 0 : (c == 1 ? 1 : 2);
        const int D = P.vol_d[l], Hh = P.vol_h[l], Ww = P.vol_w[l], C = P.vol_ch[l];
        const float ix = (pt[0] + 1.f) * 0.5f * (float)(Ww - 1), iy = (pt[1] + 1.f) * 0.5f * (float)(Hh - 1), iz = (pt[2] + 1.f) * 0.5f * (float)(D - 1);
        const float fx = floorf(ix), fy = floorf(iy), fz = floorf(iz);
        const int bx = l4 & 1, by = (l4 >> 1) & 1;
        const int xx = (int)fx + bx, yy = (int)fy + by;
        const float wxy = (bx ? ix - fx : (fx + 1.f) - ix) * (by ? iy - fy : (fy + 1.f) - iy);
        const bool inxy = xx >= 0 && xx < Ww && yy >= 0 && yy < Hh;
#pragma unroll
        for (int sl = 0; sl < 2; ++sl) {
          const int zz2 = (int)fz + sl;
          wT[sl] = wxy * (sl ? iz - fz : (fz + 1.f) - iz);
          offT[sl] = (inxy && zz2 >= 0 && zz2 < D) ? ((zz2 * Hh + yy) * Ww + xx) * C : -1;
        }
      } else if (c >= 6 && c <= 8) {
        const int k = c - 6;
        const int Ww = P.plane_w, Hh = P.plane_h;
        const float px = k == 2 ? pt[5] : pt[3], py = k == 1 ? pt[5] : pt[4];
        const float ix = ((px + 1.f) * (float)Ww - 1.f) * 0.5f, iy = ((py + 1.f) * (float)Hh - 1.f) * 0.5f;
        const float fx = floorf(ix), fy = floorf(iy);
        const int cxb = l4 & 1, cyb = (l4 >> 1) & 1;
        const int xx = (int)fx + cxb, yy = (int)fy + cyb;
        wT[0] = (cxb ? ix - fx : (fx + 1.f) - ix) * (cyb ? iy - fy : (fy + 1.f) - iy);
        offT[0] = (xx >= 0 && xx < Ww && yy >= 0 && yy < Hh) ? (yy * Ww + xx) * 32 : -1;
      } else if (c == 9) {
        const float gx = 2.0f * pu / (float)P.img_w - 1.0f, gy = 2.0f * pv / (float)P.img_h - 1.0f;
        const int cxb = l4 & 1, cyb = (l4 >> 1) & 1;
        {
          const int Ww = P.feat_w, Hh = P.feat_h;
          const float ix = (gx + 1.f) * 0.5f * (float)(Ww - 1), iy = (gy + 1.f) * 0.5f * (float)(Hh - 1);
          const float fx = floorf(ix), fy = floorf(iy);
          const int xx = (int)fx + cxb, yy = (int)fy + cyb;
          wT[0] = (cxb ? ix - fx : (fx + 1.f) - ix) * (cyb ? iy - fy : (fy + 1.f) - iy);
          offT[0] = (xx >= 0 && xx < Ww && yy >= 0 && yy < Hh) ? (yy * Ww + xx) * P.feat_ch : -1;
        }
        {
          const int Ww = P.img_w, Hh = P.img_h;
          const float ix = (gx + 1.f) * 0.5f * (float)(Ww - 1), iy = (gy + 1.f) * 0.5f * (float)(Hh - 1);
          const float fx = floorf(ix), fy = floorf(iy);
          const int xx = (int)fx + cxb, yy = (int)fy + cyb;
// ... 233 lines not shown
```

### sherf_b200/csrc/gather.cu

```cuda
#include "common.cuh"
#include "stages.cuh"
#include <cstdlib>

namespace sherf {

struct ClJobs { const float* in[8]; float* out[8]; int C[8]; long long M[8]; int blk0[9]; int vec[8]; int n; };

__global__ void __launch_bounds__(256) k_to_channels_last(const ClJobs J) {
  __shared__ float tile[32][129];
  int j = 0;
  while (j + 1 < J.n && (int)blockIdx.x >= J.blk0[j + 1]) ++j;
  const float* __restrict__ in = J.in[j];
  float* __restrict__ out = J.out[j];
  const int C = J.C[j];
  const int64_t M = J.M[j];
  const int cblocks = (C + 31) / 32;
  const int lb = (int)blockIdx.x - J.blk0[j];
  const int64_t m0 = (int64_t)(lb / cblocks) * 128;
  const int c0 = (lb % cblocks) * 32;
  const int tid = threadIdx.x;
  if (J.vec[j]) {
#pragma unroll
    for (int k = 0; k < 4; ++k) {
      const int idx = tid + 256 * k, r = idx >> 5, q = idx & 31;
// ... 210 lines not shown
#pragma unroll
      for (int t = 0; t < 4; ++t) {
        const int off = __shfl_sync(0xffffffffu, offA, 4 * k + t);
        const float w = __shfl_sync(0xffffffffu, wA, 4 * k + t);
        const float val = off >= 0 ? __ldg(base + off) : 0.f;
        acc = t == 0 ? val * w : acc + val * w;
      }
      comb[k * 96 + lane] = acc;
      if (dbgf) dbgf[k * 32 + lane] = acc;
    }
    {
      float f0 = 0.f, f1 = 0.f, rgbc = 0.f;
#pragma unroll
      for (int t = 0; t < 4; ++t) {
        const int off = __shfl_sync(0xffffffffu, offA, 12 + t);
        const float w = __shfl_sync(0xffffffffu, wA, 12 + t);
        const float v0 = off >= 0 ? __ldg(P.feat_cl + off + lane) : 0.f;
        const float v1 = off >= 0 ? __ldg(P.feat_cl + off + 32 + lane) : 0.f;
        f0 = t == 0 ? v0 * w : f0 + v0 * w;
        f1 = t == 0 ? v1 * w : f1 + v1 * w;
        const int offi = __shfl_sync(0xffffffffu, offA, 16 + t);
        const float wi = __shfl_sync(0xffffffffu, wA, 16 + t);
        const float vi = (lane < 3 && offi >= 0) ? __ldg(P.img + (size_t)lane * P.img_h * P.img_w + offi) : 0.f;
        rgbc = t == 0 ? vi * wi : rgbc + vi * wi;
      }
      const int e = lane - 3;
      const int m = e >= 0 ? e / 3 : 0, c = e >= 0 ? e - 3 * m : lane;
      const float xc = __shfl_sync(0xffffffffu, rgbc, c);
      const float enc = lane < 3 ? xc : sinf(__fadd_rn((m & 1) ? kPi2 : 0.f, __fmul_rn(xc, (float)(1 << (m >> 1)))));
      comb[0 * 96 + 32 + lane] = f0;
      comb[1 * 96 + 32 + lane] = f1;
      comb[2 * 96 + 32 + lane] = enc;
      if (dbgf) { dbgf[96 + lane] = f0; dbgf[128 + lane] = f1; dbgf[160 + lane] = enc; }
    }
    {
      int coff = 0;
#pragma unroll
      for (int l = 0; l < 3; ++l) {
        int off[8]; float w[8];
#pragma unroll
        for (int t = 0; t < 8; ++t) { off[t] = __shfl_sync(0xffffffffu, offB, 8 * l + t); w[t] = __shfl_sync(0xffffffffu, wB, 8 * l + t); }
        const float* vol = P.vol_cl[l] + lane;
#pragma unroll
        for (int gsel = 0; gsel < 3; ++gsel) {
          if (gsel <= l) {
            float acc = 0.f;
#pragma unroll
            for (int t = 0; t < 8; ++t) {
              const float val = off[t] >= 0 ? __ldg(vol + off[t] + 32 * gsel) : 0.f;
              acc += val * w[t];
            }
            f3[coff + 32 * gsel + lane] = acc;
            if (dbgf) dbgf[192 + coff + 32 * gsel + lane] = acc;
          }
        }
        coff += 32 * (l + 1);
      }
    }
    if (lane < 8) {
      float gval = 0.f;
      if (lane == 0) gval = can[0]; else if (lane == 1) gval = can[1]; else if (lane == 2) gval = can[2];
      else if (lane == 3) gval = cdir[0]; else if (lane == 4) gval = cdir[1]; else if (lane == 5) gval = cdir[2];
      P.geo[(size_t)lp * 8 + lane] = gval;
    }
    if (lane == 0 && gp < P.dbg_max) {
      if (P.dbg_vid3) P.dbg_vid3[gp] = vid3;
      if (P.dbg_can) { P.dbg_can[gp * 3] = can[0]; P.dbg_can[gp * 3 + 1] = can[1]; P.dbg_can[gp * 3 + 2] = can[2]; }
      if (P.dbg_cdir) { P.dbg_cdir[gp * 3] = cdir[0]; P.dbg_cdir[gp * 3 + 1] = cdir[1]; P.dbg_cdir[gp * 3 + 2] = cdir[2]; }
      if (P.dbg_uv) { P.dbg_uv[gp * 2] = u; P.dbg_uv[gp * 2 + 1] = v; }
    }
  }
}


__device__ __forceinline__ void grp_lexmin(float& d, int& id) {
#pragma unroll
  for (int o = 4; o > 0; o >>= 1) {
    const float od = __shfl_xor_sync(0xffffffffu, d, o);
    const int oi = __shfl_xor_sync(0xffffffffu, id, o);
    if (od < d || (od == d && oi < id)) { d = od; id = oi; }
  }
}

__device__ int nn_seeded8(const GridDesc& g, const int* __restrict__ cell_start, const float4* __restrict__ gv,
                          const float* __restrict__ t_vertices, float qx, float qy, float qz, int l8, int seed) {
  float best = dist2_xyz(qx, qy, qz, t_vertices[seed * 3], t_vertices[seed * 3 + 1], t_vertices[seed * 3 + 2]);
  int bid = seed;
  const float rb = sqrtf(best) * 1.0001f + 1.0e-4f * g.cell;
  const int x0 = min(max(grid_coord(qx - rb, g.origin[0], g.inv_cell, g.dim[0]), 0), g.dim[0] - 1);
  const int x1 = min(max(grid_coord(qx + rb, g.origin[0], g.inv_cell, g.dim[0]), 0), g.dim[0] - 1);
  const int y0 = min(max(grid_coord(qy - rb, g.origin[1], g.inv_cell, g.dim[1]), 0), g.dim[1] - 1);
  const int y1 = min(max(grid_coord(qy + rb, g.origin[1], g.inv_cell, g.dim[1]), 0), g.dim[1] - 1);
  const int z0 = min(max(grid_coord(qz - rb, g.origin[2], g.inv_cell, g.dim[2]), 0), g.dim[2] - 1);
  const int z1 = min(max(grid_coord(qz + rb, g.origin[2], g.inv_cell, g.dim[2]), 0), g.dim[2] - 1);
  const int nx = x1 - x0 + 1, ny = y1 - y0 + 1, ncells = nx * ny * (z1 - z0 + 1);
  for (int cc = l8; cc < ncells; cc += 8) {
    const int xx = x0 + cc % nx, t = cc / nx;
    const int cell = ((z0 + t / ny) * g.dim[1] + (y0 + t % ny)) * g.dim[0] + xx;
    const int b = cell_start[cell], e = cell_start[cell + 1];
    for (int k = b; k < e; ++k) {
      const float4 v = gv[k];
      const float d2 = dist2_xyz(qx, qy, qz, v.x, v.y, v.z);
      const int id = __float_as_int(v.w);
      if (d2 < best || (d2 == best && id < bid)) { best = d2; bid = id; }
    }
  }
  grp_lexmin(best, bid);
  return bid;
}

__device__ int nn_unbounded8(const GridDesc& g, const int* __restrict__ cell_start, const float4* __restrict__ gv, float qx, float qy,
                             float qz, int l8, bool active) {
  const int cx = min(max(grid_coord(qx, g.origin[0], g.inv_cell, g.dim[0]), 0), g.dim[0] - 1);
  const int cy = min(max(grid_coord(qy, g.origin[1], g.inv_cell, g.dim[1]), 0), g.dim[1] - 1);
  const int cz = min(max(grid_coord(qz, g.origin[2], g.inv_cell, g.dim[2]), 0), g.dim[2] - 1);
  float best = 3.0e38f;
  int bid = 0x7fffffff;
  (void)active;
  bool done = false;
  for (int r = 1; __any_sync(0xffffffffu, !done); r *= 2) {
    if (!done) {
      const int x0 = max(cx - r, 0), x1 = min(cx + r, g.dim[0] - 1);
      const int y0 = max(cy - r, 0), y1 = min(cy + r, g.dim[1] - 1);
      const int z0 = max(cz - r, 0), z1 = min(cz + r, g.dim[2] - 1);
      const int nx = x1 - x0 + 1, ny = y1 - y0 + 1, ncells = nx * ny * (z1 - z0 + 1);
      for (int cc = l8; cc < ncells; cc += 8) {
        const int xx = x0 + cc % nx, t = cc / nx;
        const int cell = ((z0 + t / ny) * g.dim[1] + (y0 + t % ny)) * g.dim[0] + xx;
        const int b = cell_start[cell], e = cell_start[cell + 1];
        for (int k = b; k < e; ++k) {
          const float4 v = gv[k];
          const float d2 = dist2_xyz(qx, qy, qz, v.x, v.y, v.z);
          const int id = __float_as_int(v.w);
          if (d2 < best || (d2 == best && id < bid)) { best = d2; bid = id; }
        }
      }
    }
    grp_lexmin(best, bid);
    if (!done) {
      float m = 3.0e38f;
      if (cx - r > 0) m = fminf(m, qx - (g.origin[0] + (float)(cx - r) * g.cell));
      if (cx + r < g.dim[0] - 1) m = fminf(m, (g.origin[0] + (float)(cx + r + 1) * g.cell) - qx);
      if (cy - r > 0) m = fminf(m, qy - (g.origin[1] + (float)(cy - r) * g.cell));
      if (cy + r < g.dim[1] - 1) m = fminf(m, (g.origin[1] + (float)(cy + r + 1) * g.cell) - qy);
      if (cz - r > 0) m = fminf(m, qz - (g.origin[2] + (float)(cz - r) * g.cell));
      if (cz + r < g.dim[2] - 1) m = fminf(m, (g.origin[2] + (float)(cz + r + 1) * g.cell) - qz);
      const float ms = m - 1.0e-4f * g.cell;
      if (m > 1.0e38f || (ms > 0.f && best < ms * ms)) done = true;
    }
  }
  return bid;
}

__device__ __forceinline__ void red_add4(float* p, const float4& g, float w) {
  atomicAdd(reinterpret_cast<float4*>(p), make_float4(g.x * w, g.y * w, g.z * w, g.w * w));
}

template <bool DBG, bool BWD>
__global__ void __launch_bounds__(256) k_point_gather4(const GatherParams P) {
  __shared__ FrameConst fc;
  for (int i = threadIdx.x; i < (int)(sizeof(FrameConst) / 4); i += blockDim.x) ((int*)&fc)[i] = ((const int*)P.fc)[i];
  __syncthreads();
  const int lane = threadIdx.x & 31, l8 = lane & 7, gbase = lane & 24;
  const int groups_total = gridDim.x * (blockDim.x >> 3);
  const int niter = (P.np + groups_total - 1) / groups_total;
  for (int it = 0; it < niter; ++it) {
    const int lp_raw = it * groups_total + blockIdx.x * (blockDim.x >> 3) + (threadIdx.x >> 3);
    const bool active = lp_raw < P.np;
    const int lp = active ? lp_raw : P.np - 1;
    const int64_t gp = P.p0 + lp;
    const int s = P.point_sample[gp];
    const int n = s / P.S, i = s - n * P.S;
    const float t = P.depths ? P.depths[s] : sample_depth(P.nearv[n], P.farv[n], i, P.S);
    float dray[3] = {P.dirs[n * 3], P.dirs[n * 3 + 1], P.dirs[n * 3 + 2]};
    float pw[3], q[3], vd[3];
#pragma unroll
    for (int k = 0; k < 3; ++k) pw[k] = __fsub_rn(mul_add_sep(t, dray[k], P.origins[n * 3 + k]), fc.Th_tgt[k]);
    rowvec_mat3(pw, fc.R_tgt, q);
    rowvec_mat3(dray, fc.R_tgt, vd);
    float can[3] = {q[0], q[1], q[2]}, cdir[3] = {vd[0], vd[1], vd[2]};
    apply_warp(P.T1 + P.point_vid[gp], can, cdir, true);
    const int vid3 = P.t_vertices ? nn_seeded8(fc.g3, P.g3_start, P.g3_verts, P.t_vertices, can[0], can[1], can[2], l8, P.point_vid[gp])
                                  : nn_unbounded8(fc.g3, P.g3_start, P.g3_verts, can[0], can[1], can[2], l8, active);
    float ps[3] = {can[0], can[1], can[2]}, dummy[3] = {0.f, 0.f, 0.f};
    apply_warp(P.T3 + vid3, ps, dummy, false);
    float world[3], cam[3], pix[3];
#pragma unroll
    for (int k = 0; k < 3; ++k)
      world[k] = (ps[0] * fc.Rinv_obs[k] + ps[1] * fc.Rinv_obs[3 + k] + ps[2] * fc.Rinv_obs[6 + k]) + fc.Th_obs[k];
    mat3_vec(fc.camR, world, cam);
#pragma unroll
    for (int k = 0; k < 3; ++k) cam[k] += fc.camT[k];
    mat3_vec(fc.camK, cam, pix);
    const float zz = pix[2] + 1e-5f;
    const float u = pix[0] / zz, v = pix[1] / zz;

    float cn[3];
#pragma unroll
    for (int k = 0; k < 3; ++k) cn[k] = 2.f * (can[k] - fc.twb_min[k]) / (fc.twb_max[k] - fc.twb_min[k]) - 1.f;
    const float gx = 2.0f * u / (float)P.img_w - 1.0f, gy = 2.0f * v / (float)P.img_h - 1.0f;
    float gn[3];
#pragma unroll
    for (int k = 0; k < 3; ++k) gn[k] = ((can[k] - fc.spb_min[k]) / 0.005f) / fc.out_sh[2 - k] * 2.f - 1.f;
    int offA[3], offB[3];
    float wA[3], wB[3];
#pragma unroll
    for (int sl = 0; sl < 3; ++sl) {
      const int tA = l8 + 8 * sl;
      {
        const int grp = tA >> 2;
        float ix, iy; int W, H, C;
        if (grp < 3) {
          const float px = grp == 2 ? cn[2] : cn[0], py = grp == 1 ? cn[2] : cn[1];
          W = P.plane_w; H = P.plane_h; C = 32;
          ix = ((px + 1.f) * (float)W - 1.f) * 0.5f; iy = ((py + 1.f) * (float)H - 1.f) * 0.5f;
        } else if (grp == 3) {
          W = P.feat_w; H = P.feat_h; C = P.feat_ch;
          ix = (gx + 1.f) * 0.5f * (float)(W - 1); iy = (gy + 1.f) * 0.5f * (float)(H - 1);
        } else {
          W = P.img_w; H = P.img_h; C = 1;
          ix = (gx + 1.f) * 0.5f * (float)(W - 1); iy = (gy + 1.f) * 0.5f * (float)(H - 1);
        }
        const float fx = floorf(ix), fy = floorf(iy);
        const int cxb = tA & 1, cyb = (tA >> 1) & 1;
        const int xx = (int)fx + cxb, yy = (int)fy + cyb;
        const float wx = cxb ? ix - fx : (fx + 1.f) - ix, wy = cyb ? iy - fy : (fy + 1.f) - iy;
        wA[sl] = wx * wy;
        offA[sl] = (tA < 20 && xx >= 0 && xx < W && yy >= 0 && yy < H) ? (yy * W + xx) * C : -1;
      }
      {
        const int tB = l8 + 8 * sl;
        const int l = sl;
        const int D = P.vol_d[l], H = P.vol_h[l], W = P.vol_w[l], C = P.vol_ch[l];
        const float ix = (gn[0] + 1.f) * 0.5f * (float)(W - 1), iy = (gn[1] + 1.f) * 0.5f * (float)(H - 1),
                    iz = (gn[2] + 1.f) * 0.5f * (float)(D - 1);
        const float fx = floorf(ix), fy = floorf(iy), fz = floorf(iz);
        const int bx = tB & 1, by = (tB >> 1) & 1, bz = (tB >> 2) & 1;
        const int xx = (int)fx + bx, yy = (int)fy + by, zz2 = (int)fz + bz;
        const float wx = bx ? ix - fx : (fx + 1.f) - ix, wy = by ? iy - fy : (fy + 1.f) - iy, wz = bz ? iz - fz : (fz + 1.f) - iz;
        wB[sl] = wx * wy * wz;
        offB[sl] = (xx >= 0 && xx < W && yy >= 0 && yy < H && zz2 >= 0 && zz2 < D) ? ((zz2 * H + yy) * W + xx) * C : -1;
      }
    }
    auto tapA = [&](int tix, int& off, float& w) {
      off = __shfl_sync(0xffffffffu, offA[tix >> 3], gbase + (tix & 7));
      w = __shfl_sync(0xffffffffu, wA[tix >> 3], gbase + (tix & 7));
    };
    float* comb = P.comb + (size_t)lp * 288;
    float* f3 = P.f3raw + (size_t)lp * 192;
    float* dbgf = (DBG && P.dbg_feat && gp < P.dbg_feat_max) ? P.dbg_feat + (size_t)gp * 384 : nullptr;
    const int c4 = 4 * l8;

#pragma unroll
    for (int k = 0; k < 3; ++k) {
      if (BWD) {
        if (P.g_planes_cl) {
          float* gb = P.g_planes_cl + (size_t)k * P.plane_h * P.plane_w * 32 + c4;
          const float4 g = *reinterpret_cast<const float4*>(comb + k * 96 + c4);
#pragma unroll
          for (int tp = 0; tp < 4; ++tp) {
            int off; float w;
            tapA(4 * k + tp, off, w);
            if (active && off >= 0) red_add4(gb + off, g, w);
          }
        }
// ... 145 lines not shown
```

### sherf_b200/csrc/observation.cu

```cuda
#include "common.cuh"
#include "stages.cuh"
#include <climits>

namespace sherf {

struct ObsConst {
  float bounds[6];
  int out_sh[3];
};

__global__ void k_obs_bounds(const float* __restrict__ t_vertices, int V, ObsConst* __restrict__ oc, float* __restrict__ bounds_out) {
  __shared__ float smin[3][32], smax[3][32];
  float lo[3] = {3.0e38f, 3.0e38f, 3.0e38f}, hi[3] = {-3.0e38f, -3.0e38f, -3.0e38f};
  for (int v = threadIdx.x; v < V; v += blockDim.x)
#pragma unroll
    for (int k = 0; k < 3; ++k) { const float x = t_vertices[v * 3 + k]; lo[k] = fminf(lo[k], x); hi[k] = fmaxf(hi[k], x); }
#pragma unroll
  for (int k = 0; k < 3; ++k)
    for (int o = 16; o > 0; o >>= 1) { lo[k] = fminf(lo[k], __shfl_xor_sync(0xffffffffu, lo[k], o)); hi[k] = fmaxf(hi[k], __shfl_xor_sync(0xffffffffu, hi[k], o)); }
  const int w = threadIdx.x >> 5, lane = threadIdx.x & 31;
  if (lane == 0)
#pragma unroll
    for (int k = 0; k < 3; ++k) { smin[k][w] = lo[k]; smax[k][w] = hi[k]; }
  __syncthreads();
// ... 84 lines not shown
  {
    const float* w = reinterpret_cast<const float*>(T1 + bid);
    const float a[3] = {p[0] - w[9], p[1] - w[10], p[2] - w[11]};
    float c[3];
    mat3_vec(w, a, c);
#pragma unroll
    for (int k = 0; k < 3; ++k) { c[k] = c[k] + w[12 + k]; c[k] = c[k] + w[15 + k]; c[k] = c[k] + w[18 + k]; }
    const float* Af = w + 21;
#pragma unroll
    for (int k = 0; k < 3; ++k) p[k] = (Af[4 * k] * c[0] + Af[4 * k + 1] * c[1] + Af[4 * k + 2] * c[2]) + Af[4 * k + 3];
    (void)dummy;
  }
  if (can_out) { can_out[v * 3] = p[0]; can_out[v * 3 + 1] = p[1]; can_out[v * 3 + 2] = p[2]; }
  coord[v * 4] = 0;
#pragma unroll
  for (int k = 0; k < 3; ++k)
    coord[v * 4 + 1 + k] = (int)rintf(__fdiv_rn(__fsub_rn(p[2 - k], oc->bounds[2 - k]), 0.005f));
}

__global__ void __launch_bounds__(256) k_obs_features(const float* __restrict__ uv, const unsigned char* __restrict__ vmask, int V,
                                                      const float* __restrict__ feat, int fc_, int fh, int fw, const float* __restrict__ img,
                                                      int ih, int iw, const float* __restrict__ Wp, const float* __restrict__ bp,
                                                      float* __restrict__ out) {
  __shared__ float sW[32 * 97];
  __shared__ float sx[8][96];
  for (int i = threadIdx.x; i < 32 * 96; i += blockDim.x) sW[(i / 96) * 97 + (i % 96)] = Wp[i];
  __syncthreads();
  const int lane = threadIdx.x & 31, wid = threadIdx.x >> 5;
  const int v = blockIdx.x * 8 + wid;
  if (v >= V) return;
  const float gx = 2.0f * uv[v * 2] / (float)iw - 1.0f, gy = 2.0f * uv[v * 2 + 1] / (float)ih - 1.0f;
  auto bilinear = [&](const float* __restrict__ plane, int H, int W) -> float {
    const float ix = (gx + 1.f) * 0.5f * (float)(W - 1), iy = (gy + 1.f) * 0.5f * (float)(H - 1);
    const float fx = floorf(ix), fy = floorf(iy);
    const int x0 = (int)fx, y0 = (int)fy;
    float acc = 0.f;
#pragma unroll
    for (int t = 0; t < 4; ++t) {
      const int cx = t & 1, cy = t >> 1;
      const int xx = x0 + cx, yy = y0 + cy;
      const float w = (cx ? ix - fx : (fx + 1.f) - ix) * (cy ? iy - fy : (fy + 1.f) - iy);
      const float val = (xx >= 0 && xx < W && yy >= 0 && yy < H) ? __ldg(plane + (size_t)yy * W + xx) : 0.f;
      acc = t == 0 ? val * w : acc + val * w;
    }
    return acc;
  };
  sx[wid][lane] = bilinear(feat + (size_t)lane * fh * fw, fh, fw);
  sx[wid][32 + lane] = bilinear(feat + (size_t)(32 + lane) * fh * fw, fh, fw);
  const float rgbc = lane < 3 ? bilinear(img + (size_t)lane * ih * iw, ih, iw) : 0.f;
  {
    const int e = lane - 3;
    const int m = e >= 0 ? e / 3 : 0, c = e >= 0 ? e - 3 * m : lane;
    const float xc = __shfl_sync(0xffffffffu, rgbc, c);
    sx[wid][64 + lane] = lane < 3 ? xc : sinf(__fadd_rn((m & 1) ? kPi2 : 0.f, __fmul_rn(xc, (float)(1 << (m >> 1)))));
  }
  __syncwarp();
  float acc = 0.f;
  for (int k = 0; k < 96; ++k) acc += sW[lane * 97 + k] * sx[wid][k];
  acc += bp[lane];
  out[(size_t)v * 32 + lane] = vmask[v] ? acc : 0.f;
}

size_t observation_scratch_bytes(int V, int maxcell) {
  size_t b = 4096;
  b += sizeof(FrameConst) + sizeof(ObsConst) + 512;
  b += sizeof(float) * (3 * kJoints * 16 + 3 * kJoints * 3 + 3 * kPoseFeat) + 1024;
  b += sizeof(float) * ((size_t)3 * V * 3 + (size_t)2 * V * 3 + (size_t)V * 3 + (size_t)V * 2) + 2048;
  b += sizeof(VertexWarp) * (size_t)2 * V + 512;
  b += sizeof(int) * ((size_t)2 * (maxcell + 1) + (size_t)2 * maxcell + (size_t)2 * (maxcell / 1024 + 2)) + 2048;
  b += sizeof(float4) * (size_t)2 * V + sizeof(int64_t) * 2 + (size_t)maxcell + 1024;
  b += (size_t)V + 256;
  return b;
}

int run_prepare_observation(const SherfSmplModel& smpl, const SherfObservation& ob, float* vert_feat, int32_t* coord, uint8_t* vmask_out,
                            float* bounds_out, int32_t* out_sh_host, float* can_out, void* scratch, size_t scratch_bytes, cudaStream_t st) {
  const int V = smpl.n_verts;
  constexpr int kMaxCell = 1 << 18;
  if (scratch_bytes < observation_scratch_bytes(V, kMaxCell)) { set_error("scratch arena too small for sherf_prepare_observation"); return SHERF_E_SCRATCH; }
  char* base = (char*)scratch;
  size_t off = 0;
  auto take = [&](size_t bytes) -> void* { off = (off + 255) & ~(size_t)255; void* p = base + off; off += bytes; return p; };
  { const size_t mis = ((size_t)base) & 255; if (mis) base += 256 - mis; }
  FrameTables ft;
  ft.fc = (FrameConst*)take(sizeof(FrameConst));
  ObsConst* oc = (ObsConst*)take(sizeof(ObsConst));
  ft.A = (float*)take(sizeof(float) * 3 * kJoints * 16);
  ft.joints = (float*)take(sizeof(float) * 3 * kJoints * 3);
  ft.posefeat = (float*)take(sizeof(float) * 3 * kPoseFeat);
  ft.poff = (float*)take(sizeof(float) * (size_t)3 * V * 3);
  ft.soff = (float*)take(sizeof(float) * (size_t)2 * V * 3);
  ft.verts_smpl = (float*)take(sizeof(float) * (size_t)V * 3);
  float* uv = (float*)take(sizeof(float) * (size_t)V * 2);
  ft.T1 = (VertexWarp*)take(sizeof(VertexWarp) * (size_t)V);
  ft.T3 = (VertexWarp*)take(sizeof(VertexWarp) * (size_t)V);
  ft.g1_cell_start = (int*)take(sizeof(int) * (kMaxCell + 1));
  ft.g3_cell_start = (int*)take(sizeof(int) * (kMaxCell + 1));
  ft.g_cursor = (int*)take(sizeof(int) * (size_t)2 * kMaxCell);
  ft.g_block_sums = (int*)take(sizeof(int) * (size_t)2 * (kMaxCell / 1024 + 2));
  ft.g_total = (int64_t*)take(sizeof(int64_t) * 2);
  ft.g1_verts = (float4*)take(sizeof(float4) * (size_t)V);
  ft.g3_verts = (float4*)take(sizeof(float4) * (size_t)V);
  ft.g1_occ = (unsigned char*)take(kMaxCell);
  ft.maxcell = kMaxCell;
  unsigned char* vmask = vmask_out ? vmask_out : (unsigned char*)take(V);

  SherfFrame fr;
  memset(&fr, 0, sizeof(fr));
  fr.target = ob.obs; fr.canonical = ob.canonical; fr.obs = ob.obs;
  fr.vertices = ob.obs_vertices; fr.t_vertices = ob.t_vertices;
  fr.obs_K = ob.obs_K; fr.obs_R = ob.obs_R; fr.obs_T = ob.obs_T;
  k_obs_bounds<<<1, 1024, 0, st>>>(ob.t_vertices, V, oc, bounds_out);
  SHERF_LAUNCH_CHECK();
  fr.t_world_bounds = bounds_out; fr.sp_bounds = bounds_out;
  int rc = run_prologue_frame(fr, ft, st);
  if (rc) return rc;
  rc = run_prologue_tables(smpl, fr, ft, st);
  if (rc) return rc;
  k_obs_geometry<<<ceil_div(V, 128), 128, 0, st>>>(ob.obs_vertices, V, ob.obs_R, ob.obs_T, ob.obs_K, ob.faces, ob.last_face, ob.obs.R, ob.obs.Th,
                                                  uv, vmask, ft.verts_smpl);
  SHERF_LAUNCH_CHECK();
  k_obs_canonical<<<ceil_div(V, 256), 256, 0, st>>>(ft.verts_smpl, V, ft.T1, oc, can_out, coord);
  SHERF_LAUNCH_CHECK();
  k_obs_features<<<ceil_div(V, 8), 256, 0, st>>>(uv, vmask, V, ob.obs_feat, ob.feat_ch, ob.feat_h, ob.feat_w, ob.obs_img, ob.img_h, ob.img_w,
                                                ob.proj_w, ob.proj_b, vert_feat);
  SHERF_LAUNCH_CHECK();
  SHERF_CUDA_OK(cudaMemcpyAsync(out_sh_host, oc->out_sh, sizeof(int) * 3, cudaMemcpyDeviceToHost, st));
  SHERF_CUDA_OK(cudaStreamSynchronize(st));
  return SHERF_OK;
}


constexpr int kObsBwdBlocks = 64;
__global__ void __launch_bounds__(256) k_obs_features_bwd(const float* __restrict__ uv, const unsigned char* __restrict__ vmask, int V,
                                                          const float* __restrict__ feat, int fh, int fw, const float* __restrict__ img, int ih, int iw,
                                                          const float* __restrict__ Wp, const float* __restrict__ g_out, float* __restrict__ g_Wp,
                                                          float* __restrict__ g_bp, float* __restrict__ g_feat) {
  __shared__ float sW[32 * 97];
  __shared__ float sx[8][96];
  __shared__ float sg[8][32];
  for (int i = threadIdx.x; i < 32 * 96; i += blockDim.x) sW[(i / 96) * 97 + (i % 96)] = Wp[i];
  const int lane = threadIdx.x & 31, wid = threadIdx.x >> 5;
  float accW[12], accB = 0.f;
#pragma unroll
  for (int e = 0; e < 12; ++e) accW[e] = 0.f;
  for (int v0 = blockIdx.x * 8; v0 < V; v0 += gridDim.x * 8) {
    __syncthreads();
    const int v = v0 + wid;
    float g = 0.f;
    if (v < V) {
      const float gx = 2.0f * uv[v * 2] / (float)iw - 1.0f, gy = 2.0f * uv[v * 2 + 1] / (float)ih - 1.0f;
      auto taps = [&](int H, int W, int (&xx)[4], int (&yy)[4], float (&w)[4]) {
        const float ix = (gx + 1.f) * 0.5f * (float)(W - 1), iy = (gy + 1.f) * 0.5f * (float)(H - 1);
        const float fx = floorf(ix), fy = floorf(iy);
#pragma unroll
        for (int t = 0; t < 4; ++t) {
          const int cx = t & 1, cy = t >> 1;
          xx[t] = (int)fx + cx; yy[t] = (int)fy + cy;
          w[t] = (cx ? ix - fx : (fx + 1.f) - ix) * (cy ? iy - fy : (fy + 1.f) - iy);
          if (xx[t] < 0 || xx[t] >= W || yy[t] < 0 || yy[t] >= H) w[t] = 0.f, xx[t] = 0, yy[t] = 0;
        }
      };
      int fxx[4], fyy[4], ixx[4], iyy[4];
      float fwt[4], iwt[4];
      taps(fh, fw, fxx, fyy, fwt);
      taps(ih, iw, ixx, iyy, iwt);
      auto bil = [&](const float* __restrict__ plane, int W, const int (&xx)[4], const int (&yy)[4], const float (&w)[4]) {
        float a = 0.f;
#pragma unroll
        for (int t = 0; t < 4; ++t) a += w[t] * __ldg(plane + (size_t)yy[t] * W + xx[t]);
        return a;
      };
      sx[wid][lane] = bil(feat + (size_t)lane * fh * fw, fw, fxx, fyy, fwt);
      sx[wid][32 + lane] = bil(feat + (size_t)(32 + lane) * fh * fw, fw, fxx, fyy, fwt);
      const float rgbc = lane < 3 ? bil(img + (size_t)lane * ih * iw, iw, ixx, iyy, iwt) : 0.f;
      {
        const int e = lane - 3;
        const int m = e >= 0 ? e / 3 : 0, c = e >= 0 ? e - 3 * m : lane;
        const float xc = __shfl_sync(0xffffffffu, rgbc, c);
        sx[wid][64 + lane] = lane < 3 ? xc : sinf(__fadd_rn((m & 1) ? kPi2 : 0.f, __fmul_rn(xc, (float)(1 << (m >> 1)))));
      }
      g = vmask[v] ? g_out[(size_t)v * 32 + lane] : 0.f;
      if (g_feat) {
        float d0 = 0.f, d1 = 0.f;
        for (int o = 0; o < 32; ++o) {
          const float go = __shfl_sync(0xffffffffu, g, o);
          d0 = fmaf(sW[o * 97 + lane], go, d0);
// ... 58 lines not shown
```

### sherf_b200/csrc/prologue.cu

```cuda
#include "common.cuh"
#include <limits.h>

namespace sherf {

__global__ void k_joints(const float* __restrict__ vt, const float* __restrict__ sd, const float* __restrict__ jr,
                         const float* __restrict__ b0, const float* __restrict__ b1, const float* __restrict__ b2,
                         int V, float* __restrict__ joints) {
  const int j = blockIdx.x, s = blockIdx.y;
  const float* beta = s == 0 ? b0 : (s == 1 ? b1 : b2);
  float b[10];
#pragma unroll
  for (int k = 0; k < 10; ++k) b[k] = beta[k];
  float acc[3] = {0.f, 0.f, 0.f};
  for (int v = threadIdx.x; v < V; v += blockDim.x) {
    float w = jr[(size_t)j * V + v];
    if (w != 0.f) {
#pragma unroll
      for (int c = 0; c < 3; ++c) {
        const float* row = sd + ((size_t)v * 3 + c) * 10;
        float off = 0.f;
#pragma unroll
        for (int k = 0; k < 10; ++k) off += row[k] * b[k];
        acc[c] += w * (vt[v * 3 + c] + off);
      }
// ... 151 lines not shown

__global__ void k_vertex_tables(const float* __restrict__ weights, const float* __restrict__ A, const float* __restrict__ poff,
                                const float* __restrict__ soff, const float* __restrict__ vertices, const FrameConst* __restrict__ fc,
                                int V, VertexWarp* __restrict__ T1, VertexWarp* __restrict__ T3, float* __restrict__ verts_smpl) {
  __shared__ float sA[3 * kJoints * 12];
  for (int i = threadIdx.x; i < 3 * kJoints * 12; i += blockDim.x) sA[i] = A[(i / 12) * 16 + (i % 12)];
  __syncthreads();
  const int v = blockIdx.x * blockDim.x + threadIdx.x;
  if (v >= V) return;
  float w[kJoints];
  float wsum = 0.f;
#pragma unroll
  for (int j = 0; j < kJoints; ++j) { w[j] = weights[(size_t)v * kJoints + j]; wsum += w[j]; }
  const int rows = 3 * V;
  {
    float At[12], Ab[12];
#pragma unroll
    for (int e = 0; e < 12; ++e) { At[e] = 0.f; Ab[e] = 0.f; }
#pragma unroll
    for (int j = 0; j < kJoints; ++j)
#pragma unroll
      for (int e = 0; e < 12; ++e) { At[e] += w[j] * sA[(0 * kJoints + j) * 12 + e]; Ab[e] += w[j] * sA[(1 * kJoints + j) * 12 + e]; }
    VertexWarp r;
    float R3[9] = {At[0], At[1], At[2], At[4], At[5], At[6], At[8], At[9], At[10]};
    inv3(R3, r.Rinv);
    r.t[0] = At[3]; r.t[1] = At[7]; r.t[2] = At[11];
#pragma unroll
    for (int c = 0; c < 3; ++c) {
      r.off0[c] = -poff[0 * rows + v * 3 + c];
      r.off1[c] = -soff[0 * rows + v * 3 + c];
      r.off2[c] = poff[1 * rows + v * 3 + c];
    }
#pragma unroll
    for (int e = 0; e < 12; ++e) r.Af[e] = Ab[e];
    r.pad[0] = r.pad[1] = r.pad[2] = 0.f;
    T1[v] = r;
  }
  {
    float Ab[12], Ao[12];
#pragma unroll
    for (int e = 0; e < 12; ++e) { Ab[e] = 0.f; Ao[e] = 0.f; }
#pragma unroll
    for (int j = 0; j < kJoints; ++j) {
      float wn = w[j] / wsum;
#pragma unroll
      for (int e = 0; e < 12; ++e) { Ab[e] += wn * sA[(1 * kJoints + j) * 12 + e]; Ao[e] += wn * sA[(2 * kJoints + j) * 12 + e]; }
    }
    VertexWarp r;
    float R3[9] = {Ab[0], Ab[1], Ab[2], Ab[4], Ab[5], Ab[6], Ab[8], Ab[9], Ab[10]};
    inv3(R3, r.Rinv);
    r.t[0] = Ab[3]; r.t[1] = Ab[7]; r.t[2] = Ab[11];
#pragma unroll
    for (int c = 0; c < 3; ++c) {
      r.off0[c] = -poff[1 * rows + v * 3 + c];
      r.off1[c] = soff[1 * rows + v * 3 + c];
      r.off2[c] = poff[2 * rows + v * 3 + c];
    }
#pragma unroll
    for (int e = 0; e < 12; ++e) r.Af[e] = Ao[e];
    r.pad[0] = r.pad[1] = r.pad[2] = 0.f;
    T3[v] = r;
  }
  if (verts_smpl) {
    float p[3], o[3];
#pragma unroll
    for (int c = 0; c < 3; ++c) p[c] = __fsub_rn(vertices[v * 3 + c], fc->Th_tgt[c]);
    rowvec_mat3(p, fc->R_tgt, o);
    verts_smpl[v * 3 + 0] = o[0]; verts_smpl[v * 3 + 1] = o[1]; verts_smpl[v * 3 + 2] = o[2];
  }
}

__global__ void __launch_bounds__(256) k_verts_smpl(const float* __restrict__ vertices, const FrameConst* __restrict__ fc, int V,
                                                    float* __restrict__ verts_smpl) {
  const int v = blockIdx.x * blockDim.x + threadIdx.x;
  if (v >= V) return;
  float p[3], o[3];
#pragma unroll
  for (int c = 0; c < 3; ++c) p[c] = __fsub_rn(vertices[v * 3 + c], fc->Th_tgt[c]);
  rowvec_mat3(p, fc->R_tgt, o);
  verts_smpl[v * 3 + 0] = o[0]; verts_smpl[v * 3 + 1] = o[1]; verts_smpl[v * 3 + 2] = o[2];
}

__global__ void __launch_bounds__(1024) k_grid_setup(const float* __restrict__ verts_smpl, const float* __restrict__ t_vertices, int V,
                                                      int maxcell, float min_cell, FrameConst* fc, int g0) {
  const int g = g0 + blockIdx.x;
  const float* P = g == 0 ? verts_smpl : t_vertices;
  GridDesc* gd = g == 0 ? &fc->g1 : &fc->g3;
  const int tid = threadIdx.x, nt = blockDim.x;
  __shared__ float smin[3][32], smax[3][32];
  float mn[3] = {3.0e38f, 3.0e38f, 3.0e38f}, mx[3] = {-3.0e38f, -3.0e38f, -3.0e38f};
  for (int v = tid; v < V; v += nt)
#pragma unroll
    for (int c = 0; c < 3; ++c) { float x = P[v * 3 + c]; mn[c] = fminf(mn[c], x); mx[c] = fmaxf(mx[c], x); }
#pragma unroll
  for (int c = 0; c < 3; ++c) {
    for (int o = 16; o > 0; o >>= 1) {
      mn[c] = fminf(mn[c], __shfl_xor_sync(0xffffffffu, mn[c], o));
      mx[c] = fmaxf(mx[c], __shfl_xor_sync(0xffffffffu, mx[c], o));
    }
    if ((tid & 31) == 0) { smin[c][tid >> 5] = mn[c]; smax[c][tid >> 5] = mx[c]; }
  }
  __syncthreads();
  if (tid == 0) {
    GridDesc sg;
    float lo[3], hi[3];
    for (int c = 0; c < 3; ++c) {
      lo[c] = smin[c][0]; hi[c] = smax[c][0];
      for (int w = 1; w < nt / 32; ++w) { lo[c] = fminf(lo[c], smin[c][w]); hi[c] = fmaxf(hi[c], smax[c][w]); }
    }
    float cell = min_cell;
    int d[3];
    for (int it = 0; it < 64; ++it) {
      long long n = 1;
      for (int c = 0; c < 3; ++c) { d[c] = (int)floorf((hi[c] - lo[c]) / cell) + 3; n *= d[c]; }
      if (n <= maxcell) break;
      cell *= 1.1f;
    }
    for (int c = 0; c < 3; ++c) { sg.origin[c] = lo[c] - cell; sg.dim[c] = d[c]; }
    sg.cell = cell;
    sg.inv_cell = 1.f / cell;
    sg.ncell = d[0] * d[1] * d[2];
    *gd = sg;
  }
}

__device__ __forceinline__ int vertex_cell(const GridDesc& sg, float x, float y, float z) {
  const int cx = min(max(grid_coord(x, sg.origin[0], sg.inv_cell, sg.dim[0]), 0), sg.dim[0] - 1);
  const int cy = min(max(grid_coord(y, sg.origin[1], sg.inv_cell, sg.dim[1]), 0), sg.dim[1] - 1);
  const int cz = min(max(grid_coord(z, sg.origin[2], sg.inv_cell, sg.dim[2]), 0), sg.dim[2] - 1);
  return (cz * sg.dim[1] + cy) * sg.dim[0] + cx;
}

__global__ void __launch_bounds__(256) k_grid_count(const float* __restrict__ verts_smpl, const float* __restrict__ t_vertices, int V,
                                                    const FrameConst* __restrict__ fc, int* __restrict__ counts, int maxcell, int g0) {
  const int g = g0 + blockIdx.y, v = blockIdx.x * blockDim.x + threadIdx.x;
  if (v >= V) return;
  const float* P = g == 0 ? verts_smpl : t_vertices;
  const GridDesc sg = g == 0 ? fc->g1 : fc->g3;
  atomicAdd(&counts[(size_t)g * maxcell + vertex_cell(sg, P[v * 3], P[v * 3 + 1], P[v * 3 + 2])], 1);
}

__global__ void __launch_bounds__(256) k_grid_scatter(const float* __restrict__ verts_smpl, const float* __restrict__ t_vertices, int V,
                                                      const FrameConst* __restrict__ fc, int* __restrict__ counts, int maxcell,
                                                      const int* __restrict__ g1_start, const int* __restrict__ g3_start,
                                                      float4* __restrict__ g1_verts, float4* __restrict__ g3_verts, int g0) {
  const int g = g0 + blockIdx.y, v = blockIdx.x * blockDim.x + threadIdx.x;
  if (v >= V) return;
  const float* P = g == 0 ? verts_smpl : t_vertices;
  const GridDesc sg = g == 0 ? fc->g1 : fc->g3;
  const float x = P[v * 3], y = P[v * 3 + 1], z = P[v * 3 + 2];
  const int cell = vertex_cell(sg, x, y, z);
  const int pos = (g == 0 ? g1_start : g3_start)[cell] + atomicSub(&counts[(size_t)g * maxcell + cell], 1) - 1;
  (g == 0 ? g1_verts : g3_verts)[pos] = make_float4(x, y, z, __int_as_float(v));
}

__global__ void __launch_bounds__(256) k_grid_occupancy(const FrameConst* __restrict__ fc, const int* __restrict__ g1_start,
                                                        unsigned char* __restrict__ occ) {
  const GridDesc sg = fc->g1;
  const int c = blockIdx.x * blockDim.x + threadIdx.x;
  if (c >= sg.ncell) return;
  const int x = c % sg.dim[0], t = c / sg.dim[0], y = t % sg.dim[1], z = t / sg.dim[1];
  const int x0 = max(x - 1, 0), x1 = min(x + 1, sg.dim[0] - 1);
  bool any = false;
  for (int zz = max(z - 1, 0); zz <= min(z + 1, sg.dim[2] - 1); ++zz)
    for (int yy = max(y - 1, 0); yy <= min(y + 1, sg.dim[1] - 1); ++yy) {
      const int row = (zz * sg.dim[1] + yy) * sg.dim[0];
      any |= g1_start[row + x1 + 1] > g1_start[row + x0];
    }
  occ[c] = any ? 1 : 0;
}

__global__ void k_depth_range(const float* __restrict__ nearv, const float* __restrict__ farv, int N, int S, FrameConst* fc) {
  int lo = INT_MAX, hi = INT_MIN;
  for (int n = blockIdx.x * blockDim.x + threadIdx.x; n < N; n += gridDim.x * blockDim.x) {
    float a = sample_depth(nearv[n], farv[n], 0, S), b = sample_depth(nearv[n], farv[n], S - 1, S);
    int ia = float_to_ordered(a), ib = float_to_ordered(b);
    lo = min(lo, min(ia, ib));
    hi = max(hi, max(ia, ib));
  }
  for (int o = 16; o > 0; o >>= 1) {
    lo = min(lo, __shfl_xor_sync(0xffffffffu, lo, o));
    hi = max(hi, __shfl_xor_sync(0xffffffffu, hi, o));
  }
  if ((threadIdx.x & 31) == 0) { atomicMin(&fc->dmin_bits, lo); atomicMax(&fc->dmax_bits, hi); }
}

__global__ void k_set_depth_range(FrameConst* fc, float lo, float hi) {
  fc->dmin_bits = float_to_ordered(lo);
  fc->dmax_bits = float_to_ordered(hi);
}

static Parents make_parents(const SherfSmplModel& smpl) {
  Parents p;
  for (int j = 0; j < kJoints; ++j) p.p[j] = (j == 0) ? 0 : smpl.parents[j];
  return p;
}

int run_lbs_only(const SherfSmplModel& smpl, const SherfPose& pose, float* A_out, float* joints_tmp, float* pf_tmp, cudaStream_t st) {
  k_joints<<<dim3(kJoints, 1), 256, 0, st>>>(smpl.v_template, smpl.shapedirs, smpl.j_regressor, pose.shapes, pose.shapes,
                                             pose.shapes, smpl.n_verts, joints_tmp);
  SHERF_LAUNCH_CHECK();
  k_chain<<<1, 32, 0, st>>>(pose.poses, pose.poses, pose.poses, joints_tmp, make_parents(smpl), A_out, pf_tmp);
  SHERF_LAUNCH_CHECK();
  return SHERF_OK;
}

int run_depth_range(const SherfRays& rays, FrameConst* fc, cudaStream_t st) {
  k_depth_range<<<min(ceil_div(rays.n_rays, 256), 1184), 256, 0, st>>>(rays.near_, rays.far_, rays.n_rays, rays.n_samples, fc);
  SHERF_LAUNCH_CHECK();
  return SHERF_OK;
}

static int build_grid(int g, const SherfFrame& fr, const FrameTables& ft, int V, cudaStream_t st) {
  int* counts = ft.g_cursor + (size_t)g * ft.maxcell;
  int* bsums = ft.g_block_sums + (size_t)g * (ft.maxcell / 1024 + 2);
  k_grid_setup<<<1, 1024, 0, st>>>(ft.verts_smpl, fr.t_vertices, V, ft.maxcell, 0.0505f, ft.fc, g);
  SHERF_LAUNCH_CHECK();
  SHERF_CUDA_OK(cudaMemsetAsync(counts, 0, sizeof(int) * (size_t)ft.maxcell, st));
  k_grid_count<<<dim3(ceil_div(V, 256), 1), 256, 0, st>>>(ft.verts_smpl, fr.t_vertices, V, ft.fc, ft.g_cursor, ft.maxcell, g);
  SHERF_LAUNCH_CHECK();
  int rc = run_exclusive_scan(counts, ft.maxcell, bsums, g == 0 ? ft.g1_cell_start : ft.g3_cell_start, ft.g_total + g, st);
  if (rc) return rc;
  k_grid_scatter<<<dim3(ceil_div(V, 256), 1), 256, 0, st>>>(ft.verts_smpl, fr.t_vertices, V, ft.fc, ft.g_cursor, ft.maxcell, ft.g1_cell_start,
                                                           ft.g3_cell_start, ft.g1_verts, ft.g3_verts, g);
  SHERF_LAUNCH_CHECK();
  if (g == 0) {
    k_grid_occupancy<<<ceil_div(ft.maxcell, 256), 256, 0, st>>>(ft.fc, ft.g1_cell_start, ft.g1_occ);
    SHERF_LAUNCH_CHECK();
  }
  return SHERF_OK;
}

int run_prologue_frame(const SherfFrame& fr, const FrameTables& ft, cudaStream_t st) {
  SHERF_CUDA_OK(cudaMemsetAsync(ft.fc, 0, sizeof(FrameConst), st));
  k_frame_const<<<1, 32, 0, st>>>(fr, make_float3((float)fr.out_sh[0], (float)fr.out_sh[1], (float)fr.out_sh[2]), ft.fc);
  SHERF_LAUNCH_CHECK();
  return SHERF_OK;
}

int run_prologue_cull(const SherfSmplModel& smpl, const SherfFrame& fr, const SherfRays& rays, const SherfOptions& opts,
                      const FrameTables& ft, cudaStream_t st) {
  const int V = smpl.n_verts;
  k_verts_smpl<<<ceil_div(V, 256), 256, 0, st>>>(fr.vertices, ft.fc, V, ft.verts_smpl);
  SHERF_LAUNCH_CHECK();
  int rc = build_grid(0, fr, ft, V, st);
  if (rc) return rc;
  if (opts.use_external_clamp) {
    k_set_depth_range<<<1, 1, 0, st>>>(ft.fc, opts.depth_clamp_min, opts.depth_clamp_max);
    SHERF_LAUNCH_CHECK();
  } else {
    rc = run_depth_range(rays, ft.fc, st);
    if (rc) return rc;
  }
  return SHERF_OK;
}

int run_prologue_tables(const SherfSmplModel& smpl, const SherfFrame& fr, const FrameTables& ft, cudaStream_t st) {
  const int V = smpl.n_verts;
  k_joints<<<dim3(kJoints, 3), 256, 0, st>>>(smpl.v_template, smpl.shapedirs, smpl.j_regressor, fr.target.shapes,
                                             fr.canonical.shapes, fr.obs.shapes, V, ft.joints);
  SHERF_LAUNCH_CHECK();
  k_chain<<<3, 32, 0, st>>>(fr.target.poses, fr.canonical.poses, fr.obs.poses, ft.joints, make_parents(smpl), ft.A, ft.posefeat);
  SHERF_LAUNCH_CHECK();
  k_offsets<<<ceil_div(3 * V, 8), 256, 0, st>>>(smpl.posedirs, smpl.shapedirs, ft.posefeat, fr.target.shapes, fr.obs.shapes,
                                                3 * V, ft.poff, ft.soff);
  SHERF_LAUNCH_CHECK();
  k_vertex_tables<<<ceil_div(V, 128), 128, 0, st>>>(smpl.weights, ft.A, ft.poff, ft.soff, fr.vertices, ft.fc, V, ft.T1, ft.T3, nullptr);
  SHERF_LAUNCH_CHECK();
  return build_grid(1, fr, ft, V, st);
}

}
```

### sherf_b200/csrc/stages.cuh

```cuda
#pragma once
#include "common.cuh"

namespace sherf {

struct DevCount { const int64_t* total; int64_t p0; int cap; };
__device__ __forceinline__ int resolve_np(int np_host, const DevCount& dc) {
  if (!dc.total) return np_host;
  const int64_t r = *dc.total - dc.p0;
  return r <= 0 ? 0 : (r > dc.cap ? dc.cap : (int)r);
}

struct GatherParams {
  const float *origins, *dirs, *nearv, *farv;
  int S;
  const float* depths;
  const int *point_sample, *point_vid;
  int64_t p0; int np;
  DevCount dc;
  const FrameConst* fc;
  const VertexWarp *T1, *T3;
  const int* g3_start; const float4* g3_verts;
  const float* t_vertices;
  const float* planes_cl; int plane_h, plane_w;
  const float* feat_cl; int feat_h, feat_w, feat_ch;
  const float* img; int img_h, img_w;
  const float* vol_cl[3]; int vol_ch[3]; int vol_d[3], vol_h[3], vol_w[3];
  float* comb;
  float* f3raw;
  float* geo;
  float* g_planes_cl; float* g_feat_cl; float* g_vol_cl[3];
  int* dbg_vid3; float *dbg_can, *dbg_cdir, *dbg_uv, *dbg_feat; int64_t dbg_max, dbg_feat_max;
};

int run_to_channels_last_multi(int n, const float* const* in, float* const* out, const int* C, const int64_t* M, cudaStream_t st);
int run_point_gather(const GatherParams& P, cudaStream_t st);
int run_point_scatter(const GatherParams& P, cudaStream_t st);
int run_cull(const SherfRays& rays, int S, const float* depths, const FrameTables& ft, int* sample_vid, int* ray_count, int* block_sums,
             int* ray_start, int64_t* total_dev, int* point_sample, int* point_vid, cudaStream_t st, int write_all = 1);

struct ChunkBuffers {
  int cap;
  float *comb;
  float *f3raw;
  float *geo;
  float *tok;
  float *ln;
  float *qkv;
  float *att;
  float *tok2;
  float *ffh;
  float *tok3;
  float *x;
  float *h1, *h2;
  float *hb;
  float *fv;
  float *vh;
};
size_t chunk_buffer_floats(int cap);
void carve_chunk_buffers(float* base, int cap, ChunkBuffers& cb);

struct PackedLayer { const float* wt; const float* bias; int K, N, kp, np; };
struct PackedWeights {
  PackedLayer proj, reproj, qkv, attn_out, ff1, ff2, pts[8], feature, views;
};
size_t packed_weight_floats();
int run_pack_weights(const SherfWeights& w, float* base, PackedWeights& pw, cudaStream_t st);

struct CanonLayer { const float* hi; const float* lo; const float* bias; int N, K, Np, nchunks; };
struct CanonWeights { CanonLayer proj, reproj, qkv, attn_out, ff1, ff2, pts[8], feature, views; };
size_t canonical_weight_floats();
int run_pack_canonical(const SherfWeights& w, float* base, CanonWeights& cw, cudaStream_t st);
int launch_umma_linear(int prec, const CanonLayer& L, const float* A, int lda, float* Y, int ldy, int M, int act, cudaStream_t st,
                       const float* Res, int ldr, int ygroup, int ygstride, const float* ln_w = nullptr, const float* ln_b = nullptr,
                       float* Y2 = nullptr, int ldy2 = 0);
int launch_simt_linear(const PackedLayer& L, const float* A, int lda, float* Y, int ldy, int M, int act, cudaStream_t st,
                       const float* Res, int ldr, int ygroup, int ygstride);
struct CanonBwdWeights { CanonLayer views, feature, pts[8] , pts5x, ff2, ff1, attn_out, qkv, reproj, proj; };
size_t canonical_bwd_weight_floats();
int run_pack_canonical_bwd(const SherfWeights& w, float* base, CanonBwdWeights& cb, cudaStream_t st);
int launch_umma_dx(const CanonLayer& L, const float* dY, int lda, float* dX, int ldx, int M, cudaStream_t st, const float* Mask = nullptr,
                   int ldm = 0, int accum = 0, int agroup = 0, int agstride = 0);
size_t spconv_canon_floats();
int run_pack_spconv(const float* W, int cout, int cin, int mode, float* buf, CanonLayer& L, cudaStream_t st);
int launch_umma_spconv(const CanonLayer& L, const float* X, int kin, const int* rowtab, const int* Mdev, int Mcap, float* Ypart, int nsplit,
                       cudaStream_t st);
constexpr int kGradWMaxSplits = 1024;
int launch_umma_grad_w(const float* dY, int lda, int N, const float* X, int ldb, int K, int M, float* part, int* splits_out, cudaStream_t st,
                       int agroup = 0, int agstride = 0);

struct FusedChunk { uint32_t w_off; uint32_t w_bytes; uint16_t src; uint16_t kg0; uint16_t nkg; uint16_t layer; uint16_t first; uint16_t last; };
struct FusedSchedule { FusedChunk ch[44]; uint16_t layer_np[10]; uint16_t pad[2]; };
struct PpPlan { uint32_t w_off[23]; const unsigned char* blob; const float* bias; unsigned char* xp; unsigned char* vp; };
struct FusedPlan { FusedSchedule sch; const unsigned char* blob; const float* bias; const float* xf_blob; const float* ff_blob; const PpPlan* pp;
                   const unsigned char* xb_blob;  const unsigned char* fr_blob;  };
size_t pp_blob_bytes();
size_t pp_xv_bytes(int cap);
int run_pack_pp(const SherfWeights& w, unsigned char* blob, float* bias, PpPlan& plan, cudaStream_t st);
int run_pack_xv(const float* x, int ldx, const float* fv, int ldfv, int np, unsigned char* xp, unsigned char* vp, cudaStream_t st);
int run_decoder_pp(const PpPlan& plan, const SherfWeights& w, const unsigned char* xp, const unsigned char* vp, float* sigma, float* rgb, int np,
                   cudaStream_t st, DevCount dc = DevCount{nullptr, 0, 0});
size_t fused_blob_bytes();
extern long long* g_fused_trace;
int run_pack_fused_plan(const SherfWeights& w, unsigned char* blob, float* bias, FusedPlan& plan, cudaStream_t st);
int run_decoder_fused_plan(int prec, const FusedPlan& plan, const float* X, int ldx, const float* fv, int ldfv, float* sigma, float* rgb,
                           const float* rgb_w, const float* rgb_b, int np, cudaStream_t st);
// ... 86 lines not shown
```

Baseline: 5.584 billion.

## Precompute per-subcell nearest-neighbor candidate lists for cull and KNN lookups

```diff
diff --git a/include/sherf_b200.h b/include/sherf_b200.h
--- a/include/sherf_b200.h
+++ b/include/sherf_b200.h
@@ -274,6 +274,7 @@
 SHERF_API void sherf_set_profiling(int enabled);
 SHERF_API float sherf_last_stage_ms(int stage);
 SHERF_API float sherf_last_host_us(int part);
+SHERF_API int sherf_nn_list_stats(double* out);
 
 #ifdef __cplusplus
 }
diff --git a/sherf_b200/_lib.py b/sherf_b200/_lib.py
--- a/sherf_b200/_lib.py
+++ b/sherf_b200/_lib.py
@@ -101,7 +101,7 @@
 
 
 EXPORTS = ['sherf_render_backward_after_forward', 'sherf_sparse_encoder_train_scratch_bytes', 'sherf_sparse_encode_train', 'sherf_sparse_encode_backward', 'sherf_prepare_observation_backward', 'sherf_backward_scratch_bytes', 'sherf_render_backward', 'sherf_smpl_vertices', 'sherf_count_survivors', 'sherf_observation_scratch_bytes', 'sherf_prepare_observation', 'sherf_debug_set_trace', 'sherf_sparse_encoder_scratch_bytes', 'sherf_sparse_encode', 'sherf_generate_rays', 'sherf_debug_sample_importance', 'sherf_debug_linear', 'sherf_scratch_bytes', 'sherf_render_forward', 'sherf_lbs_transforms', 'sherf_depth_range', 'sherf_last_error',
-           'sherf_abi_version', 'sherf_last_launch_count', 'sherf_last_importance_point_count', 'sherf_set_profiling', 'sherf_last_stage_ms', 'sherf_last_host_us']
+           'sherf_abi_version', 'sherf_last_launch_count', 'sherf_last_importance_point_count', 'sherf_set_profiling', 'sherf_last_stage_ms', 'sherf_last_host_us', 'sherf_nn_list_stats']
 
 _lib = None
 
@@ -183,6 +183,8 @@
     lib.sherf_set_profiling.argtypes = [C.c_int]
     lib.sherf_last_stage_ms.restype = C.c_float
     lib.sherf_last_stage_ms.argtypes = [C.c_int]
+    lib.sherf_nn_list_stats.restype = C.c_int
+    lib.sherf_nn_list_stats.argtypes = [C.POINTER(C.c_double)]
     lib.sherf_last_host_us.restype = C.c_float
     lib.sherf_last_host_us.argtypes = [C.c_int]
     if lib.sherf_abi_version() != ABI_VERSION:
diff --git a/sherf_b200/csrc/api.cu b/sherf_b200/csrc/api.cu
--- a/sherf_b200/csrc/api.cu
+++ b/sherf_b200/csrc/api.cu
@@ -16,6 +16,7 @@
 static thread_local int64_t g_last_fine_points = 0;
 static thread_local int g_profiling = 0;
 static thread_local float g_stage_ms[8] = {0, 0, 0, 0, 0, 0, 0, 0};
+static thread_local FrameTables g_last_ft{};
 static thread_local float g_host_us[4] = {0, 0, 0, 0};
 static inline double now_us() { return std::chrono::duration<double, std::micro>(std::chrono::steady_clock::now().time_since_epoch()).count(); }
 
@@ -27,6 +28,16 @@
 }
 
 constexpr int kMaxCell = 1 << 18;
+
+bool nn_lists_enabled() {
+  const char* e = getenv("SHERF_NN_LEGACY");
+  return !(e && atoi(e) != 0);
+}
+int nn_list_cap() {
+  const char* e = getenv("SHERF_NN_LIST_CAP");
+  const int k = e ? atoi(e) : kNnlCap;
+  return k < 1 ? 1 : (k > kNnlCap ? kNnlCap : k);
+}
 static size_t chunk_cap_limit() {
   static size_t cap = 0;
   if (!cap) {
@@ -91,6 +102,16 @@
   ft.g3_verts = a.take<float4>(V);
   ft.g1_occ = a.take<unsigned char>(kMaxCell);
   ft.maxcell = kMaxCell;
+  ft.nnl_on = nn_lists_enabled() ? 1 : 0;
+  ft.nnl_cap = nn_list_cap();
+  ft.nnl_count = a.take<int>(4);
+  ft.nnl_cand = a.take<unsigned char>((size_t)kMaxCell * kNnlSub3);
+  for (int g = 0; g < 2; ++g) {
+    ft.nnl_slot[g] = a.take<int>(kMaxCell);
+    ft.nnl_slot_cell[g] = a.take<int>(kNnlSlots);
+    ft.nnl_len[g] = a.take<int>((size_t)kNnlSlots * kNnlSub3);
+    ft.nnl_ent[g] = a.take<float4>((size_t)kNnlSlots * kNnlSub3 * kNnlCap);
+  }
   L.lbs_joints = a.take<float>(kJoints * 3);
   L.lbs_pf = a.take<float>(kPoseFeat);
   L.planes_cl = a.take<float>((size_t)3 * sc.plane_ch * sc.plane_h * sc.plane_w);
@@ -217,6 +238,7 @@
   G.point_sample = L.point_sample; G.point_vid = L.point_vid; G.p0 = 0; G.np = 0; G.dc = DevCount{nullptr, 0, 0};
   G.fc = L.ft.fc; G.T1 = L.ft.T1; G.T3 = L.ft.T3; G.g3_start = L.ft.g3_cell_start; G.g3_verts = L.ft.g3_verts;
   G.t_vertices = getenv("SHERF_KNN3_UNSEEDED") ? nullptr : frame.t_vertices;
+  G.nl3 = L.ft.lists(1);
   G.planes_cl = L.planes_cl; G.plane_h = scene.plane_h; G.plane_w = scene.plane_w;
   G.feat_cl = L.feat_cl; G.feat_h = scene.feat_h; G.feat_w = scene.feat_w; G.feat_ch = scene.feat_ch;
   G.img = scene.obs_img; G.img_h = scene.img_h; G.img_w = scene.img_w;
@@ -276,6 +298,31 @@
 void sherf_set_profiling(int enabled) { g_profiling = enabled; }
 float sherf_last_stage_ms(int stage) { return (stage >= 0 && stage < 8) ? g_stage_ms[stage] : 0.f; }
 float sherf_last_host_us(int part) { return (part >= 0 && part < 4) ? g_host_us[part] : 0.f; }
+
+int sherf_nn_list_stats(double* out) {
+  if (!out || !g_last_ft.nnl_on) { set_error("the last forward on this thread built no candidate lists"); return SHERF_E_INVALID; }
+  const FrameTables& ft = g_last_ft;
+  SHERF_CUDA_OK(cudaDeviceSynchronize());
+  int cnt[4];
+  SHERF_CUDA_OK(cudaMemcpy(cnt, ft.nnl_count, sizeof(cnt), cudaMemcpyDeviceToHost));
+  out[0] = cnt[2];
+  std::vector<int> len((size_t)kNnlSlots * kNnlSub3);
+  for (int g = 0; g < 2; ++g) {
+    const int nsub = (cnt[g] < kNnlSlots ? cnt[g] : kNnlSlots) * kNnlSub3;
+    SHERF_CUDA_OK(cudaMemcpy(len.data(), ft.nnl_len[g], sizeof(int) * (size_t)nsub, cudaMemcpyDeviceToHost));
+    double sum = 0.0, mx = 0.0, over = 0.0;
+    for (int i = 0; i < nsub; ++i) {
+      if (len[i] < 0) over += 1.0;
+      else { sum += len[i]; mx = len[i] > mx ? len[i] : mx; }
+    }
+    out[1 + 4 * g] = nsub;
+    out[2 + 4 * g] = nsub > over ? sum / (nsub - over) : 0.0;
+    out[3 + 4 * g] = mx;
+    out[4 + 4 * g] = nsub ? over / nsub : 0.0;
+  }
+  out[9] = ft.nnl_cap;
+  return SHERF_OK;
+}
 
 size_t sherf_scratch_bytes(const SherfScene* scene, int32_t n_rays, int32_t n_samples, int32_t n_importance, int32_t n_verts) {
   if (!scene || n_rays <= 0 || n_samples < 2 || n_importance < 0 || n_verts <= 0) return 0;
@@ -524,6 +571,7 @@
   }
   tm.finish();
   g_last_launches = g_launches.n;
+  g_last_ft = L.ft;
   { const double t_exit = now_us(); g_host_us[0] = (float)(t_sync0 - t_enter); g_host_us[1] = (float)(t_sync1 - t_sync0); g_host_us[2] = (float)(t_exit - t_sync1); g_host_us[3] = (float)(t_exit - t_enter); }
   return SHERF_OK;
 }
@@ -635,6 +683,7 @@
     carve_bwd_chunk(B.chunk, B.bcap, bc);
     GatherParams G;
     fill_gather_params(G, *rays, *frame, *scene, L);
+    G.nl3 = NnLists{nullptr, nullptr, nullptr, nullptr};
     for (int64_t p0 = 0; p0 < P; p0 += B.bcap) {
       const int np = (int)((P - p0 < B.bcap) ? (P - p0) : B.bcap);
       RC(run_backward_chunk(*weights, pw, cw, cbw, gw, G, bc, np, p0, L.rgb, B.dsig, B.drgb, st));
diff --git a/sherf_b200/csrc/common.cuh b/sherf_b200/csrc/common.cuh
--- a/sherf_b200/csrc/common.cuh
+++ b/sherf_b200/csrc/common.cuh
@@ -18,6 +18,37 @@
   int dim[3];
   int ncell;
 };
+
+constexpr int kNnlSub = 2;
+constexpr int kNnlSub3 = kNnlSub * kNnlSub * kNnlSub;
+constexpr int kNnlCap = 64;
+constexpr int kNnlSlots = 6144;
+
+struct NnLists {
+  const int* slot;
+  const int* len;
+  const float4* ent;
+  const unsigned char* cand;
+};
+
+__device__ __forceinline__ bool nnl_cell(const GridDesc& g, float qx, float qy, float qz, int& cell, int& sub) {
+  const float tx = (qx - g.origin[0]) * g.inv_cell, ty = (qy - g.origin[1]) * g.inv_cell, tz = (qz - g.origin[2]) * g.inv_cell;
+  const int cx = (int)floorf(tx), cy = (int)floorf(ty), cz = (int)floorf(tz);
+  if (cx < 0 || cx >= g.dim[0] || cy < 0 || cy >= g.dim[1] || cz < 0 || cz >= g.dim[2]) return false;
+  cell = (cz * g.dim[1] + cy) * g.dim[0] + cx;
+  const int sx = min((int)((tx - (float)cx) * (float)kNnlSub), kNnlSub - 1);
+  const int sy = min((int)((ty - (float)cy) * (float)kNnlSub), kNnlSub - 1);
+  const int sz = min((int)((tz - (float)cz) * (float)kNnlSub), kNnlSub - 1);
+  sub = (sz * kNnlSub + sy) * kNnlSub + sx;
+  return true;
+}
+
+__device__ __forceinline__ int nnl_index(const GridDesc& g, const int* __restrict__ slot, float qx, float qy, float qz) {
+  int cell, sub;
+  if (!nnl_cell(g, qx, qy, qz, cell, sub)) return -1;
+  const int sl = slot[cell];
+  return sl < 0 ? sl - 1 : sl * kNnlSub3 + sub;
+}
 
 struct __align__(16) VertexWarp {
   float Rinv[9];
@@ -123,7 +154,20 @@
   float4* g3_verts;
   unsigned char* g1_occ;
   int maxcell;
+  int nnl_on;
+  int nnl_cap;
+  int* nnl_slot[2];
+  int* nnl_slot_cell[2];
+  int* nnl_count;
+  int* nnl_len[2];
+  float4* nnl_ent[2];
+  unsigned char* nnl_cand;
+  NnLists lists(int g) const {
+    return nnl_on ? NnLists{nnl_slot[g], nnl_len[g], nnl_ent[g], g == 0 ? nnl_cand : nullptr} : NnLists{nullptr, nullptr, nullptr, nullptr};
+  }
 };
+bool nn_lists_enabled();
+int nn_list_cap();
 
 int run_prologue_frame(const SherfFrame& frame, const FrameTables& ft, cudaStream_t st);
 int run_prologue_cull(const SherfSmplModel& smpl, const SherfFrame& frame, const SherfRays& rays, const SherfOptions& opts,
diff --git a/sherf_b200/csrc/cull.cu b/sherf_b200/csrc/cull.cu
--- a/sherf_b200/csrc/cull.cu
+++ b/sherf_b200/csrc/cull.cu
@@ -33,7 +33,7 @@
                                                          const FrameConst* __restrict__ fcp, const unsigned char* __restrict__ occ,
                                                          const float* __restrict__ depths, int* __restrict__ sample_vid,
                                                          int* __restrict__ ray_count, int* __restrict__ queue, int* __restrict__ queue_count,
-                                                         int write_all) {
+                                                         int write_all, const NnLists nl) {
   __shared__ FrameConst fc;
   for (int i = threadIdx.x; i < (int)(sizeof(FrameConst) / 4); i += blockDim.x) ((int*)&fc)[i] = ((const int*)fcp)[i];
   __syncthreads();
@@ -76,10 +76,15 @@
       if (t < t0 || t > t1) { sample_vid[(size_t)n * S + i] = -1; }
       else {
       cull_query(fc, origins, dirs, n, t, q);
-      const int cx = grid_coord(q[0], g.origin[0], g.inv_cell, g.dim[0]);
-      const int cy = grid_coord(q[1], g.origin[1], g.inv_cell, g.dim[1]);
-      const int cz = grid_coord(q[2], g.origin[2], g.inv_cell, g.dim[2]);
-      cand = cx >= 0 && cx < g.dim[0] && cy >= 0 && cy < g.dim[1] && cz >= 0 && cz < g.dim[2] && occ[(cz * g.dim[1] + cy) * g.dim[0] + cx];
+      if (nl.cand) {
+        int cell, sub;
+        cand = nnl_cell(g, q[0], q[1], q[2], cell, sub) && nl.cand[cell * kNnlSub3 + sub];
+      } else {
+        const int cx = grid_coord(q[0], g.origin[0], g.inv_cell, g.dim[0]);
+        const int cy = grid_coord(q[1], g.origin[1], g.inv_cell, g.dim[1]);
+        const int cz = grid_coord(q[2], g.origin[2], g.inv_cell, g.dim[2]);
+        cand = cx >= 0 && cx < g.dim[0] && cy >= 0 && cy < g.dim[1] && cz >= 0 && cz < g.dim[2] && occ[(cz * g.dim[1] + cy) * g.dim[0] + cx];
+      }
       if (!cand) sample_vid[(size_t)n * S + i] = -1;
       }
     }
@@ -93,29 +98,44 @@
   }
 }
 
-__global__ void __launch_bounds__(256) k_cull_search(const float* __restrict__ origins, const float* __restrict__ dirs,
+__global__ void __launch_bounds__(256, 4) k_cull_search(const float* __restrict__ origins, const float* __restrict__ dirs,
                                                      const float* __restrict__ nearv, const float* __restrict__ farv, int S,
                                                      const FrameConst* __restrict__ fcp, const int* __restrict__ cell_start,
                                                      const float4* __restrict__ gv, float thr, const float* __restrict__ depths,
                                                      const int* __restrict__ queue, const int* __restrict__ queue_count,
-                                                     int* __restrict__ sample_vid, int* __restrict__ ray_count) {
+                                                     int* __restrict__ sample_vid, int* __restrict__ ray_count, const NnLists nl,
+                                                     int* __restrict__ cand_out) {
   __shared__ FrameConst fc;
   for (int i = threadIdx.x; i < (int)(sizeof(FrameConst) / 4); i += blockDim.x) ((int*)&fc)[i] = ((const int*)fcp)[i];
   __syncthreads();
   const GridDesc& g = fc.g1;
   const int count = *queue_count;
+  if (cand_out && blockIdx.x == 0 && threadIdx.x == 0) *cand_out = count;
   for (int j = blockIdx.x * blockDim.x + threadIdx.x; j < count; j += gridDim.x * blockDim.x) {
     const int s = queue[j];
     const int n = s / S, i = s - n * S;
     const float t = depths ? depths[s] : sample_depth(nearv[n], farv[n], i, S);
     float q[3];
     cull_query(fc, origins, dirs, n, t, q);
-    const int cx = grid_coord(q[0], g.origin[0], g.inv_cell, g.dim[0]);
-    const int cy = grid_coord(q[1], g.origin[1], g.inv_cell, g.dim[1]);
-    const int cz = grid_coord(q[2], g.origin[2], g.inv_cell, g.dim[2]);
     float best = 3.0e38f;
     int bid = 0x7fffffff;
-    nn_27(g, cell_start, gv, q[0], q[1], q[2], cx, cy, cz, best, bid);
+    const float qx = q[0], qy = q[1], qz = q[2];
+    const int li = nl.slot ? nnl_index(g, nl.slot, qx, qy, qz) : -1;
+    const int ln = li >= 0 ? nl.len[li] : -1;
+    if (ln >= 0) {
+      const float4* e = nl.ent + (size_t)li * kNnlCap;
+      for (int k = 0; k < ln; ++k) {
+        const float4 v = e[k];
+        const float d2 = dist2_xyz(qx, qy, qz, v.x, v.y, v.z);
+        const int id = __float_as_int(v.w);
+        if (d2 < best || (d2 == best && id < bid)) { best = d2; bid = id; }
+      }
+    } else {
+      const int cx = grid_coord(q[0], g.origin[0], g.inv_cell, g.dim[0]);
+      const int cy = grid_coord(q[1], g.origin[1], g.inv_cell, g.dim[1]);
+      const int cz = grid_coord(q[2], g.origin[2], g.inv_cell, g.dim[2]);
+      nn_27(g, cell_start, gv, qx, qy, qz, cx, cy, cz, best, bid);
+    }
     const int vid = best < thr ? bid : -1;
     sample_vid[s] = vid;
     if (vid >= 0) atomicAdd(&ray_count[n], 1);
@@ -211,10 +231,10 @@
   int* queue_count = reinterpret_cast<int*>(total_dev);
   SHERF_CUDA_OK(cudaMemsetAsync(queue_count, 0, sizeof(int), st));
   k_cull_candidates<<<ceil_div(N, 8), 256, 0, st>>>(rays.origins, rays.dirs, rays.near_, rays.far_, N, S, ft.fc, ft.g1_occ, depths,
-                                                    sample_vid, ray_count, queue, queue_count, write_all);
+                                                    sample_vid, ray_count, queue, queue_count, write_all, ft.lists(0));
   SHERF_LAUNCH_CHECK();
   k_cull_search<<<148 * 8, 256, 0, st>>>(rays.origins, rays.dirs, rays.near_, rays.far_, S, ft.fc, ft.g1_cell_start, ft.g1_verts, thr, depths,
-                                         queue, queue_count, sample_vid, ray_count);
+                                         queue, queue_count, sample_vid, ray_count, ft.lists(0), ft.nnl_on ? ft.nnl_count + 2 : nullptr);
   SHERF_LAUNCH_CHECK();
   RC_SCAN(run_exclusive_scan(ray_count, N, block_sums, ray_start, total_dev, st));
   k_compact<<<ceil_div(N, 8), 256, 0, st>>>(sample_vid, ray_start, N, S, point_sample, point_vid);
diff --git a/sherf_b200/csrc/front_fused.cu b/sherf_b200/csrc/front_fused.cu
--- a/sherf_b200/csrc/front_fused.cu
+++ b/sherf_b200/csrc/front_fused.cu
@@ -65,7 +65,23 @@
 }
 
 __device__ __forceinline__ int fr_nn_seeded4(const GridDesc& g, const int* __restrict__ cell_start, const float4* __restrict__ gv,
-                                             const float* __restrict__ t_vertices, float qx, float qy, float qz, int l4, int seed) {
+                                             const NnLists& nl, const float* __restrict__ t_vertices, float qx, float qy, float qz, int l4,
+                                             int seed) {
+  const int li = nl.slot ? nnl_index(g, nl.slot, qx, qy, qz) : -1;
+  const int ln = li >= 0 ? nl.len[li] : -1;
+  if (ln > 0) {
+    float best = 3.0e38f;
+    int bid = 0x7fffffff;
+    const float4* e = nl.ent + (size_t)li * kNnlCap;
+    for (int k = l4; k < ln; k += 4) {
+      const float4 v = e[k];
+      const float d2 = dist2_xyz(qx, qy, qz, v.x, v.y, v.z);
+      const int id = __float_as_int(v.w);
+      if (d2 < best || (d2 == best && id < bid)) { best = d2; bid = id; }
+    }
+    fr_grp_lexmin(best, bid);
+    return bid;
+  }
   float best = dist2_xyz(qx, qy, qz, t_vertices[seed * 3], t_vertices[seed * 3 + 1], t_vertices[seed * 3 + 2]);
   int bid = seed;
   const float rb = sqrtf(best) * 1.0001f + 1.0e-4f * g.cell;
@@ -178,7 +194,7 @@
       float cn[3] = {q[0], q[1], q[2]}, cdir[3] = {vd[0], vd[1], vd[2]};
       const int vid1 = P.point_vid[gp];
       if (!(a.knock & 8)) fr_apply_warp(P.T1 + vid1, cn, cdir, true);
-      const int vid3 = (a.knock & 1) ? vid1 : fr_nn_seeded4(fc.g3, P.g3_start, P.g3_verts, P.t_vertices, cn[0], cn[1], cn[2], l4, vid1);
+      const int vid3 = (a.knock & 1) ? vid1 : fr_nn_seeded4(fc.g3, P.g3_start, P.g3_verts, P.nl3, P.t_vertices, cn[0], cn[1], cn[2], l4, vid1);
       float ps[3] = {cn[0], cn[1], cn[2]}, dummy[3] = {0.f, 0.f, 0.f};
       fr_apply_warp(P.T3 + vid3, ps, dummy, false);
       float world[3], cam[3], pix[3];
diff --git a/sherf_b200/csrc/gather.cu b/sherf_b200/csrc/gather.cu
--- a/sherf_b200/csrc/gather.cu
+++ b/sherf_b200/csrc/gather.cu
@@ -316,8 +316,23 @@
   }
 }
 
-__device__ int nn_seeded8(const GridDesc& g, const int* __restrict__ cell_start, const float4* __restrict__ gv,
+__device__ int nn_seeded8(const GridDesc& g, const int* __restrict__ cell_start, const float4* __restrict__ gv, const NnLists& nl,
                           const float* __restrict__ t_vertices, float qx, float qy, float qz, int l8, int seed) {
+  const int li = nl.slot ? nnl_index(g, nl.slot, qx, qy, qz) : -1;
+  const int ln = li >= 0 ? nl.len[li] : -1;
+  if (ln > 0) {
+    float best = 3.0e38f;
+    int bid = 0x7fffffff;
+    const float4* e = nl.ent + (size_t)li * kNnlCap;
+    for (int k = l8; k < ln; k += 8) {
+      const float4 v = e[k];
+      const float d2 = dist2_xyz(qx, qy, qz, v.x, v.y, v.z);
+      const int id = __float_as_int(v.w);
+      if (d2 < best || (d2 == best && id < bid)) { best = d2; bid = id; }
+    }
+    grp_lexmin(best, bid);
+    return bid;
+  }
   float best = dist2_xyz(qx, qy, qz, t_vertices[seed * 3], t_vertices[seed * 3 + 1], t_vertices[seed * 3 + 2]);
   int bid = seed;
   const float rb = sqrtf(best) * 1.0001f + 1.0e-4f * g.cell;
@@ -414,7 +429,7 @@
     rowvec_mat3(dray, fc.R_tgt, vd);
     float can[3] = {q[0], q[1], q[2]}, cdir[3] = {vd[0], vd[1], vd[2]};
     apply_warp(P.T1 + P.point_vid[gp], can, cdir, true);
-    const int vid3 = P.t_vertices ? nn_seeded8(fc.g3, P.g3_start, P.g3_verts, P.t_vertices, can[0], can[1], can[2], l8, P.point_vid[gp])
+    const int vid3 = P.t_vertices ? nn_seeded8(fc.g3, P.g3_start, P.g3_verts, BWD ? NnLists{nullptr, nullptr, nullptr, nullptr} : P.nl3, P.t_vertices, can[0], can[1], can[2], l8, P.point_vid[gp])
                                   : nn_unbounded8(fc.g3, P.g3_start, P.g3_verts, can[0], can[1], can[2], l8, active);
     float ps[3] = {can[0], can[1], can[2]}, dummy[3] = {0.f, 0.f, 0.f};
     apply_warp(P.T3 + vid3, ps, dummy, false);
diff --git a/sherf_b200/csrc/observation.cu b/sherf_b200/csrc/observation.cu
--- a/sherf_b200/csrc/observation.cu
+++ b/sherf_b200/csrc/observation.cu
@@ -190,7 +190,7 @@
   size_t off = 0;
   auto take = [&](size_t bytes) -> void* { off = (off + 255) & ~(size_t)255; void* p = base + off; off += bytes; return p; };
   { const size_t mis = ((size_t)base) & 255; if (mis) base += 256 - mis; }
-  FrameTables ft;
+  FrameTables ft{};
   ft.fc = (FrameConst*)take(sizeof(FrameConst));
   ObsConst* oc = (ObsConst*)take(sizeof(ObsConst));
   ft.A = (float*)take(sizeof(float) * 3 * kJoints * 16);
@@ -211,6 +211,7 @@
   ft.g3_verts = (float4*)take(sizeof(float4) * (size_t)V);
   ft.g1_occ = (unsigned char*)take(kMaxCell);
   ft.maxcell = kMaxCell;
+  ft.nnl_on = 0;
   unsigned char* vmask = vmask_out ? vmask_out : (unsigned char*)take(V);
 
   SherfFrame fr;
diff --git a/sherf_b200/csrc/prologue.cu b/sherf_b200/csrc/prologue.cu
--- a/sherf_b200/csrc/prologue.cu
+++ b/sherf_b200/csrc/prologue.cu
@@ -257,8 +257,9 @@
 }
 
 __global__ void __launch_bounds__(1024) k_grid_setup(const float* __restrict__ verts_smpl, const float* __restrict__ t_vertices, int V,
-                                                      int maxcell, float min_cell, FrameConst* fc, int g0) {
+                                                      int maxcell, float min_cell, FrameConst* fc, int g0, int* nslots) {
   const int g = g0 + blockIdx.x;
+  if (nslots && threadIdx.x == 0) nslots[g] = 0;
   const float* P = g == 0 ? verts_smpl : t_vertices;
   GridDesc* gd = g == 0 ? &fc->g1 : &fc->g3;
   const int tid = threadIdx.x, nt = blockDim.x;
@@ -329,9 +330,10 @@
   (g == 0 ? g1_verts : g3_verts)[pos] = make_float4(x, y, z, __int_as_float(v));
 }
 
-__global__ void __launch_bounds__(256) k_grid_occupancy(const FrameConst* __restrict__ fc, const int* __restrict__ g1_start,
-                                                        unsigned char* __restrict__ occ) {
-  const GridDesc sg = fc->g1;
+__global__ void __launch_bounds__(256) k_grid_occupancy(const FrameConst* __restrict__ fc, int g, const int* __restrict__ start,
+                                                        unsigned char* __restrict__ occ, int* __restrict__ slot, int* __restrict__ slot_cell,
+                                                        int* __restrict__ nslots, unsigned char* __restrict__ cand) {
+  const GridDesc sg = g == 0 ? fc->g1 : fc->g3;
   const int c = blockIdx.x * blockDim.x + threadIdx.x;
   if (c >= sg.ncell) return;
   const int x = c % sg.dim[0], t = c / sg.dim[0], y = t % sg.dim[1], z = t / sg.dim[1];
@@ -340,9 +342,119 @@
   for (int zz = max(z - 1, 0); zz <= min(z + 1, sg.dim[2] - 1); ++zz)
     for (int yy = max(y - 1, 0); yy <= min(y + 1, sg.dim[1] - 1); ++yy) {
       const int row = (zz * sg.dim[1] + yy) * sg.dim[0];
-      any |= g1_start[row + x1 + 1] > g1_start[row + x0];
-    }
-  occ[c] = any ? 1 : 0;
+      any |= start[row + x1 + 1] > start[row + x0];
+    }
+  if (occ) occ[c] = any ? 1 : 0;
+  if (cand) *reinterpret_cast<uint2*>(cand + (size_t)c * kNnlSub3) = any ? make_uint2(0x01010101u, 0x01010101u) : make_uint2(0u, 0u);
+  if (slot) {
+    const unsigned act = __activemask(), m = __ballot_sync(act, any);
+    const int lane = threadIdx.x & 31, leader = __ffs(act) - 1;
+    int base = 0;
+    if (lane == leader && m) base = atomicAdd(nslots, __popc(m));
+    base = __shfl_sync(act, base, leader);
+    int s = -1;
+    if (any) {
+      s = base + __popc(m & ((1u << lane) - 1u));
+      if (s < kNnlSlots) slot_cell[s] = c;
+      else s = -2;
+    }
+    slot[c] = s;
+  }
+}
+
+__global__ void __launch_bounds__(256) k_nnl_build(const FrameConst* __restrict__ fc, int g, const int* __restrict__ start,
+                                                   const float4* __restrict__ gv, const int* __restrict__ slot_cell,
+                                                   const int* __restrict__ nslots, int cap, float cut, int* __restrict__ len,
+                                                   float4* __restrict__ ent, unsigned char* __restrict__ cand) {
+  static_assert(kNnlSub == 2, "one bit per axis selects the sub-cell");
+  const GridDesc sg = g == 0 ? fc->g1 : fc->g3;
+  const int lane = threadIdx.x & 31;
+  const int ns = min(*nslots, kNnlSlots);
+  const float f = sg.cell * 0.5f, eps = 1.0e-4f * sg.cell;
+  for (int sl = (blockIdx.x * blockDim.x + threadIdx.x) >> 5; sl < ns; sl += (gridDim.x * blockDim.x) >> 5) {
+    const int c = slot_cell[sl];
+    const int cx = c % sg.dim[0], t = c / sg.dim[0], cy = t % sg.dim[1], cz = t / sg.dim[1];
+    const int cc[3] = {cx, cy, cz};
+    float lo[3][2], hi[3][2], ctr[3][2];
+#pragma unroll
+    for (int k = 0; k < 3; ++k)
+#pragma unroll
+      for (int h = 0; h < 2; ++h) {
+        lo[k][h] = sg.origin[k] + (float)cc[k] * sg.cell + (float)h * f - eps;
+        hi[k][h] = lo[k][h] + f + 2.f * eps;
+        ctr[k][h] = 0.5f * (lo[k][h] + hi[k][h]);
+      }
+    float dc[8];
+#pragma unroll
+    for (int i = 0; i < 8; ++i) dc[i] = 3.0e38f;
+    for (int zz = max(cz - 1, 0); zz <= min(cz + 1, sg.dim[2] - 1); ++zz)
+      for (int yy = max(cy - 1, 0); yy <= min(cy + 1, sg.dim[1] - 1); ++yy) {
+        const int row = (zz * sg.dim[1] + yy) * sg.dim[0];
+        const int b = start[row + max(cx - 1, 0)], e = start[row + min(cx + 1, sg.dim[0] - 1) + 1];
+        for (int k = b + lane; k < e; k += 32) {
+          const float4 v = gv[k];
+          float d[3][2];
+#pragma unroll
+          for (int h = 0; h < 2; ++h) {
+            d[0][h] = (v.x - ctr[0][h]) * (v.x - ctr[0][h]);
+            d[1][h] = (v.y - ctr[1][h]) * (v.y - ctr[1][h]);
+            d[2][h] = (v.z - ctr[2][h]) * (v.z - ctr[2][h]);
+          }
+#pragma unroll
+          for (int i = 0; i < 8; ++i) dc[i] = fminf(dc[i], d[0][i & 1] + d[1][(i >> 1) & 1] + d[2][i >> 2]);
+        }
+      }
+    float lim2[8];
+    int rmax = 0, rbits = 0;
+#pragma unroll
+    for (int i = 0; i < 8; ++i) {
+      float x = dc[i];
+      for (int o = 16; o > 0; o >>= 1) x = fminf(x, __shfl_xor_sync(0xffffffffu, x, o));
+      float lim = (sqrtf(x) + 1.7320508f * (0.5f * f + eps)) * 1.0001f + eps;
+      if (cut > 0.f) lim = fminf(lim, cut);
+      const int r = lim < 0.999f * sg.cell ? 1 : (lim < 1.999f * sg.cell ? 2 : 0);
+      rmax = max(rmax, r);
+      rbits |= r > 0 ? 1 << i : 0;
+      lim2[i] = r > 0 ? lim * lim : -1.f;
+    }
+    int n[8];
+#pragma unroll
+    for (int i = 0; i < 8; ++i) n[i] = 0;
+    float4* out = ent + (size_t)sl * kNnlSub3 * kNnlCap;
+    for (int zz = max(cz - rmax, 0); zz <= min(cz + rmax, sg.dim[2] - 1); ++zz)
+      for (int yy = max(cy - rmax, 0); yy <= min(cy + rmax, sg.dim[1] - 1); ++yy) {
+        const int row = (zz * sg.dim[1] + yy) * sg.dim[0];
+        const int b = start[row + max(cx - rmax, 0)], e = start[row + min(cx + rmax, sg.dim[0] - 1) + 1];
+        for (int k0 = b; k0 < e; k0 += 32) {
+          const int k = k0 + lane;
+          const float4 v = k < e ? gv[k] : make_float4(3.0e38f, 3.0e38f, 3.0e38f, 0.f);
+          float o[3][2];
+#pragma unroll
+          for (int h = 0; h < 2; ++h) {
+            const float ox = fmaxf(fmaxf(lo[0][h] - v.x, v.x - hi[0][h]), 0.f);
+            const float oy = fmaxf(fmaxf(lo[1][h] - v.y, v.y - hi[1][h]), 0.f);
+            const float oz = fmaxf(fmaxf(lo[2][h] - v.z, v.z - hi[2][h]), 0.f);
+            o[0][h] = ox * ox; o[1][h] = oy * oy; o[2][h] = oz * oz;
+          }
+#pragma unroll
+          for (int i = 0; i < 8; ++i) {
+            const bool take = k < e && o[0][i & 1] + o[1][(i >> 1) & 1] + o[2][i >> 2] <= lim2[i];
+            const unsigned m = __ballot_sync(0xffffffffu, take);
+            const int pos = n[i] + __popc(m & ((1u << lane) - 1u));
+            if (take && pos < cap) out[i * kNnlCap + pos] = v;
+            n[i] += __popc(m);
+          }
+        }
+      }
+#pragma unroll
+    for (int i = 0; i < 8; ++i) {
+      if (lane == i) {
+        const int l = ((rbits >> i) & 1) && n[i] <= cap ? n[i] : -1;
+        len[sl * kNnlSub3 + i] = l;
+        if (cand) cand[(size_t)c * kNnlSub3 + i] = l != 0;
+      }
+    }
+  }
 }
 
 __global__ void k_depth_range(const float* __restrict__ nearv, const float* __restrict__ farv, int N, int S, FrameConst* fc) {
@@ -389,7 +501,8 @@
 static int build_grid(int g, const SherfFrame& fr, const FrameTables& ft, int V, cudaStream_t st) {
   int* counts = ft.g_cursor + (size_t)g * ft.maxcell;
   int* bsums = ft.g_block_sums + (size_t)g * (ft.maxcell / 1024 + 2);
-  k_grid_setup<<<1, 1024, 0, st>>>(ft.verts_smpl, fr.t_vertices, V, ft.maxcell, 0.0505f, ft.fc, g);
+  const bool lists = ft.nnl_on != 0;
+  k_grid_setup<<<1, 1024, 0, st>>>(ft.verts_smpl, fr.t_vertices, V, ft.maxcell, 0.0505f, ft.fc, g, lists ? ft.nnl_count : nullptr);
   SHERF_LAUNCH_CHECK();
   SHERF_CUDA_OK(cudaMemsetAsync(counts, 0, sizeof(int) * (size_t)ft.maxcell, st));
   k_grid_count<<<dim3(ceil_div(V, 256), 1), 256, 0, st>>>(ft.verts_smpl, fr.t_vertices, V, ft.fc, ft.g_cursor, ft.maxcell, g);
@@ -399,8 +512,17 @@
   k_grid_scatter<<<dim3(ceil_div(V, 256), 1), 256, 0, st>>>(ft.verts_smpl, fr.t_vertices, V, ft.fc, ft.g_cursor, ft.maxcell, ft.g1_cell_start,
                                                            ft.g3_cell_start, ft.g1_verts, ft.g3_verts, g);
   SHERF_LAUNCH_CHECK();
-  if (g == 0) {
-    k_grid_occupancy<<<ceil_div(ft.maxcell, 256), 256, 0, st>>>(ft.fc, ft.g1_cell_start, ft.g1_occ);
+  if (g == 0 || lists) {
+    k_grid_occupancy<<<ceil_div(ft.maxcell, 256), 256, 0, st>>>(ft.fc, g, g == 0 ? ft.g1_cell_start : ft.g3_cell_start, g == 0 ? ft.g1_occ : nullptr,
+                                                                lists ? ft.nnl_slot[g] : nullptr, ft.nnl_slot_cell[g], ft.nnl_count + g,
+                                                                lists && g == 0 ? ft.nnl_cand : nullptr);
+    SHERF_LAUNCH_CHECK();
+  }
+  if (lists) {
+    const float cut = g == 0 ? 0.05f * 1.0001f + 1.0e-5f : 0.f;
+    k_nnl_build<<<148 * 8, 256, 0, st>>>(ft.fc, g, g == 0 ? ft.g1_cell_start : ft.g3_cell_start, g == 0 ? ft.g1_verts : ft.g3_verts,
+                                         ft.nnl_slot_cell[g], ft.nnl_count + g, ft.nnl_cap, cut, ft.nnl_len[g], ft.nnl_ent[g],
+                                         g == 0 ? ft.nnl_cand : nullptr);
     SHERF_LAUNCH_CHECK();
   }
   return SHERF_OK;
diff --git a/sherf_b200/csrc/stages.cuh b/sherf_b200/csrc/stages.cuh
--- a/sherf_b200/csrc/stages.cuh
+++ b/sherf_b200/csrc/stages.cuh
@@ -21,6 +21,7 @@
   const VertexWarp *T1, *T3;
   const int* g3_start; const float4* g3_verts;
   const float* t_vertices;
+  NnLists nl3;
   const float* planes_cl; int plane_h, plane_w;
   const float* feat_cl; int feat_h, feat_w, feat_ch;
   const float* img; int img_h, img_w;
```

Measured after the change: 5.877 billion (median of 6 runs). +5.2%, better.
